# micahvista/VACmap

Hardware: AMD Instinct MI355X
Metric: aligned Gbp/s (whole node) + reads/s, 15 kb ONT-shape reads vs hg38-size ref, 1/2/4/8 MI355X (higher is better)
Workload: dtype i16/i32 DP + f64 chains

## Files before the change

### include/vacmapx.h

```cpp
#ifndef VACMAPX_H
#define VACMAPX_H
#include <stdint.h>
#ifdef __cplusplus
extern "C" {
#endif

typedef enum vm_status {
    VM_OK = 0,
    VM_ERR_ARG = -1,
    VM_ERR_NO_DEVICE = -2,
    VM_ERR_NO_CTX = -3,
    VM_ERR_OOM = -4,
    VM_ERR_IO = -5,
    VM_ERR_HIP = -6,
    VM_ERR_UNSUPPORTED = -7,
    VM_READ_RAISED = -10,
    VM_READ_CAPACITY = -20,
    VM_READ_FASTPATH = -21,
    VM_READ_UNSUPPORTED = -22
} vm_status;

enum { VM_MODE_H = 0, VM_MODE_L = 1, VM_MODE_S = 2, VM_MODE_R = 3,
       VM_MODE_ASM = 4 };

// ... 45 lines not shown
int vm_index_blob_count(const vm_index*);
int vm_index_blob(const vm_index*, int i, void** dev_ptr, int64_t* bytes);
int vm_index_meta_size(const vm_index*, int64_t* bytes);
int vm_index_meta_get(const vm_index*, void* buf, int64_t bytes);
int vm_index_from_meta(vm_ctx*, const void* buf, int64_t bytes, vm_index** out);

int vm_sketch_batch(vm_ctx*, int k, int w, int64_t n, const char* seqs, const int64_t* offsets,
                    uint64_t** hash, int32_t** pos, int8_t** strand, int64_t** off);
int vm_map_batch(vm_ctx*, const vm_index*, int check_num, int mid_occ, int64_t n, const char* seqs,
                 const int64_t* offsets, int64_t** anchors, int64_t** anchor_off);
int vm_map(vm_ctx*, const vm_index*, const char* seq, int64_t len, int check_num, int mid_occ, int64_t** anchors, int64_t* n);

typedef struct vm_chains_out {
    int32_t* need_reverse;
    int32_t* mapq;
    double* score;
    int32_t* fast_used;
    int64_t* read_path_off;
    int64_t* path_off;
    int64_t* path_anchors;
    double* S; int64_t* P; int64_t* S_arg; int64_t* gmax; int64_t* opcount;
} vm_chains_out;
int vm_chain_global_batch(vm_ctx*, const vm_params*, int kmersize, int64_t n, const int64_t* anchors,
                          const int64_t* anchor_off, const int64_t* readlens, int want_raw, vm_chains_out* out);
void vm_chains_out_free(vm_chains_out*);

typedef struct vm_local_out {
    int32_t* status;
    int32_t* variant;
    double* score;
    int64_t* chain_off;
    int64_t* chain;
    int64_t* raw_off;
    int64_t* raw;
} vm_local_out;
int vm_local_chain_batch(vm_ctx*, const vm_index*, const vm_params*, int64_t n, const char* seqs, const int64_t* offsets,
                         const int64_t* read_path_off, const int64_t* path_off, const int64_t* path_anchors, vm_local_out* out);
void vm_local_out_free(vm_local_out*);

typedef struct vm_linked_out {
    int64_t gmax, n_hot, n_cold, opcount; double cold_max;
    double* S; int64_t* P; int64_t* S_arg_hot;
    int32_t carry_status, saved; int64_t n_carry; double* carry_S; int64_t* carry_P; int64_t* carry_rows; double carry_g_max_scores; int64_t carry_prereadloc;
} vm_linked_out;
int vm_chain_linked(vm_ctx*, int which, int kmersize, double skipcost, int maxdiff, int maxgap, int64_t n, const int64_t* rows, int64_t n_pre,
                    const double* pre_S, const int64_t* pre_P, double g_max_scores, int64_t g_max_index, int64_t prereadloc, vm_linked_out* out);
void vm_linked_out_free(vm_linked_out*);

typedef struct vm_score { int32_t match, mismatch, o1, e1, o2, e2; } vm_score;
int vm_k_cigar_batch(vm_ctx*, const vm_score*, int eqx, int64_t n, const char* t, const int64_t* t_off, const char* q,
                     const int64_t* q_off, char** cigars, int64_t** cigar_off, int32_t** scores);
int vm_k_cigar_batch_banded(vm_ctx*, const vm_score*, int eqx, int64_t n, const char* t, const int64_t* t_off, const char* q,
                            const int64_t* q_off, char** cigars, int64_t** cigar_off, int32_t** band_flag, int64_t* stats);
int vm_k_extend_batch(vm_ctx*, int match, int mismatch, int o, int e, int bw, int zdrop, int64_t n, const char* t,
                      const int64_t* t_off, const char* q, const int64_t* q_off, int32_t** t_e, int32_t** q_e, int32_t** score);
typedef struct vm_cigar_out { char* cigar; int32_t q_e, t_e, score; } vm_cigar_out;
int vm_k_cigar(vm_ctx*, const char* t, int64_t tl, const char* q, int64_t ql, const vm_score* sc, int bw, int zdrop,
               int eqx, vm_cigar_out* out);
int vm_edit_distance_batch(vm_ctx*, int64_t n, const char* q, const int64_t* q_off, const char* t, const int64_t* t_off,
                           int64_t** dist);
int64_t vm_edit_distance(vm_ctx*, const char* q, int64_t ql, const char* t, int64_t tl);
int vm_edit_distance_bound_batch(vm_ctx*, int tier, int64_t n, const char* q, const int64_t* q_off, const char* t, const int64_t* t_off,
                                 int64_t** bound);

typedef struct vm_record {
    int32_t read_idx;
    int32_t contig;
    int32_t strand;
    int32_t mapq;
    int64_t q_st, q_en;
    int64_t r_st, r_en;
    int64_t cigar_off, cigar_len;
} vm_record;

typedef struct vm_batch_stats {
    int64_t n_reads, read_bases, n_minimizers, n_hits, n_anchors, n_local_hits, n_local_anchors;
    int64_t n_segments, n_ed_problems, ed_cells, n_ext_problems, ext_cells, n_dp_problems, dp_cells;
    int64_t n_records, cigar_bytes, aligned_bases, n_unmapped, n_failed;
    int64_t dp_string_bytes;
    double ms_total;
    double ms_stage[16];
    double ms_gapfill_fill;
    double ms_gapfill_trace;
    int64_t n_gapfill_launches;
    int64_t n_ed_full;
    int64_t n_ed_tier2;
    int64_t n_ed_tier1;
    int64_t n_dp_redo;
    int64_t dp_redo_tb_bytes;
    double ms_local_seed;
    double ms_cluster;
    int64_t n_host_syncs;
    int64_t n_local_general;
    int64_t n_ext_retries;
    int64_t n_batch_retries;
    int64_t n_dp_redo_wide;
    int64_t n_dp_redo_full;
} vm_batch_stats;

int vm_align_batch(vm_ctx*, const vm_index*, const vm_params*, int64_t n_reads, const char* seqs, const int64_t* offsets,
                   vm_record** recs, int64_t* n_recs, char** cigar_blob, int32_t* status_per_read, vm_batch_stats* stats);
typedef struct vm_reads vm_reads;
int vm_reads_upload(vm_ctx*, int64_t n_reads, const char* seqs, const int64_t* offsets, vm_reads** out);
int vm_reads_reupload(vm_ctx*, vm_reads*, int64_t n_reads, const char* seqs, const int64_t* offsets);
void vm_reads_free(vm_reads*);
int vm_align_resident(vm_ctx*, const vm_index*, const vm_params*, const vm_reads*, vm_record** recs, int64_t* n_recs,
                      char** cigar_blob, int32_t* status_per_read, vm_batch_stats* stats);

int vm_align_asm(vm_ctx*, const vm_index*, const vm_params* p, const char* contig, int64_t len, int64_t split_len, int64_t batch_anchors, int64_t window,
                 vm_record** recs, int64_t* n_recs, char** cigar_blob, int32_t* status);

int vm_align_trace(vm_ctx*, const vm_index*, const vm_params*, int64_t n_reads, const char* seqs, const int64_t* offsets, int stage,
                   int64_t** rows, int64_t** row_off);

typedef struct vm_sam_opts {
    int32_t md, shortcs, cigar2cg, markunbalancetra, hardclip, fakecigar;
    const char* rg_id;
    int32_t asm_mode;
} vm_sam_opts;
int vm_sam_emit(const vm_index*, const vm_sam_opts*, int64_t n_reads, const char* names, const int64_t* name_off, const char* seqs, const int64_t* seq_off,
                const char* quals, const int64_t* qual_off, const char* comments, const int64_t* com_off, const vm_record* recs, int64_t n_recs,
                const char* cigar_blob, const int32_t* status, int nthreads, char** text, int64_t** text_off, int64_t* n_lines, int64_t* n_skipped);
int vm_sam_emit_device(vm_ctx*, const vm_index*, const vm_sam_opts*, int64_t n_reads, const char* names, const int64_t* name_off, const char* seqs,
                       const int64_t* seq_off, const char* quals, const int64_t* qual_off, const vm_record* recs, int64_t n_recs, const char* cigar_blob,
                       const int32_t* status, char** text, int64_t** text_off, int64_t* n_lines, int64_t* n_skipped);
int vm_sam_emit_device_times(vm_ctx*, double* seconds3);
int64_t vm_blob_gather(const char* blob, const int64_t* off, const int64_t* idx, int64_t n, char* out, int64_t* out_off);
int64_t vm_blob_write_parts_mmap(int fd, int64_t file_off, const char* const* blobs, const int64_t* const* offs, const int32_t* part, const int64_t* idx, int64_t n, int nthreads);
int64_t vm_blob_gather_parts(const char* const* blobs, const int64_t* const* offs, const int32_t* part, const int64_t* idx, int64_t n, char* out);
void* vm_pinned_alloc(int64_t bytes, int device);
void vm_pinned_free(void* p);
int64_t vm_blob_write_parts(int fd, const char* const* blobs, const int64_t* const* offs, const int32_t* part, const int64_t* idx, int64_t n);
typedef struct vm_fastx vm_fastx;
int vm_fastx_open(const char* path, vm_fastx** out);
int vm_fastx_open_range(const char* path, int64_t begin, int64_t end, vm_fastx** out);
void vm_fastx_close(vm_fastx*);
int64_t vm_fastx_read(vm_fastx*, int64_t max_reads, int64_t max_bases, char** names, int64_t** name_off, char** seqs, int64_t** seq_off, char** quals,
                      int64_t** qual_off, char** comments, int64_t** com_off);

typedef struct vm_bam_writer vm_bam_writer;
int vm_bam_writer_create(vm_ctx*, const char* sam_header, int64_t len, vm_bam_writer** out);
void vm_bam_writer_free(vm_bam_writer*);
int vm_bam_header(vm_bam_writer*, char** out, int64_t* n);
int vm_bam_encode(vm_bam_writer*, const char* sam, int64_t len, char** out, int64_t* n);
int vm_bam_compress_parts(vm_bam_writer*, const char* const* blobs, const int64_t* const* offs, const int32_t* part, const int64_t* idx, int64_t n,
                          char** out, int64_t* n_out);
int vm_bgzf_compress(vm_ctx*, const void* in, int64_t n, char** out, int64_t* n_out);

int vm_bgzf_decompress(vm_ctx*, const void* in, int64_t n, char** out, int64_t* n_out);
typedef struct vm_bam_reader vm_bam_reader;
// ... 26 lines not shown
```

### vacmap_amd/csrc/k_dp.hip

```cpp
#include "vmx_device.h"
#include "vmx_kernels.h"

__device__ __forceinline__ int vmx_tcode(uint8_t c) { return c < 4 ? (int)c : 6; }


__global__ void k_encode(const char* __restrict__ in, uint8_t* __restrict__ out, int64_t n) {
    int64_t i = (int64_t)blockIdx.x * blockDim.x + threadIdx.x;
    int64_t stride = (int64_t)gridDim.x * blockDim.x;
    for (; i < n; i += stride) out[i] = vmx_code((uint8_t)in[i]);
}

#define VMX_EXT_RING 512
__global__ void __launch_bounds__(64) k_extend(const uint8_t* __restrict__ tcodes, const int64_t* __restrict__ t_off,
                                               const uint8_t* __restrict__ qcodes, const int64_t* __restrict__ q_off, int n_prob,
                                               int match, int mismatch, int o, int e, int bw_in, int zdrop,
                                               int32_t* __restrict__ out_te, int32_t* __restrict__ out_qe, int32_t* __restrict__ out_sc, const int32_t* __restrict__ n_ptr) {
    if (n_ptr) n_prob = *n_ptr;
    __shared__ int sH[3][VMX_EXT_RING];
    __shared__ int sE[2][VMX_EXT_RING];
    __shared__ int sF[2][VMX_EXT_RING];
    const int lane = vmx_lane();
    const int RM = VMX_EXT_RING - 1;
    for (int p = blockIdx.x; p < n_prob; p += gridDim.x) {
        const uint8_t* T = tcodes + t_off[p];
// ... 396 lines not shown
                if (ns == 2) VMX_ADW_RUN(2); else if (ns == 3) VMX_ADW_RUN(3); else VMX_ADW_RUN(4);
#undef VMX_ADW_RUN
                keepX = gX > 0 && vmx_ad_proven(scX, tlX0, qlX0, gX, match, o1, e1, o2, e2);
                keepY = gY > 0 && vmx_ad_proven(scY, tlY0, qlY0, gY, match, o1, e1, o2, e2);
            }
            if (lane == 0) {
                if (keepX) out_score[pX] = VMX_PK_FLAG;
                if (keepY) out_score[pY] = VMX_PK_FLAG;
                const int kept = (int)keepX + (int)keepY, full = 1 + (int)(pY >= 0) - kept;
                if (kept) atomicAdd(redo_cnt + 6, kept);
                if (full) atomicAdd(redo_cnt + 7, full);
            }
            if (!keepX || (pY >= 0 && !keepY)) __syncthreads();
            if (!keepX) vmx_gapfill_fill_one<SCORE>(tcodes, qcodes, probs, pX, match, mismatch, o1, e1, o2, e2, tb_pool, bnd_pool, out_score, lane, VMX_PK_FLAG, redo_pool);
            if (pY >= 0 && !keepY) vmx_gapfill_fill_one<SCORE>(tcodes, qcodes, probs, pY, match, mismatch, o1, e1, o2, e2, tb_pool, bnd_pool, out_score, lane, VMX_PK_FLAG, redo_pool);
        }
    }
    while (true) {
        int q0;
        if (order) { int v = 0; if (lane == 0) v = atomicAdd(counter, 4); q0 = vmx_bcast0(v); }
        else { q0 = static_next; static_next += 4 * (int)gridDim.x; }
        if (q0 >= n_prob) break;
        const int qg = q0 + (lane >> 4);
        const int pg = qg < n_prob ? (order ? order[qg] : qg) : -1;
        bool x4 = false, skip = false;
        {
            vmx_dp_prob pr; pr.tl = 0; pr.ql = 0; pr.t_off = 0; pr.q_off = 0; pr.tb_off = 0; pr.bnd_off = 0;
            if (pg >= 0) pr = probs[pg];
            skip = redo_pass && pg >= 0 && VMX_REDO_PK(pr.tl, pr.ql);
            x4 = pg >= 0 && !skip && pr.tl > 0 && pr.ql > 0 && VMX_DP16X4_OK(pr.tl, pr.ql);
            if (!SCORE && x4 && (lane & 15) == 0) out_score[pg] = 0;
            if (__any(x4))
                vmx_gapfill_fill16x4<SCORE>(tcodes + pr.t_off, qcodes + pr.q_off, x4 ? pr.tl : 0, x4 ? pr.ql : 0, match, mismatch, o1, e1, o2, e2, vmx_tb_ptr(tb_pool, redo_pool, pr.tb_off),
                                            bnd_pool + pr.bnd_off, &out_score[pg < 0 ? 0 : pg], lane);
        }
        for (int gk = 0; gk < 4; ++gk) {
            const int p = vmx_readlane(pg, 16 * gk);
            if (p < 0 || vmx_readlane((int)(x4 || skip), 16 * gk)) continue;
            vmx_gapfill_fill_one<SCORE>(tcodes, qcodes, probs, p, match, mismatch, o1, e1, o2, e2, tb_pool, bnd_pool, out_score, lane, 0, redo_pool);
        }
    }
}

__device__ __forceinline__ void vmx_gapfill_ad_pass(const uint8_t* __restrict__ tcodes, const uint8_t* __restrict__ qcodes, vmx_dp_prob* __restrict__ probs, int n_prob,
                                                   int match, int mismatch, int o1, int e1, int o2, int e2, uint8_t* __restrict__ tb_pool, int32_t* __restrict__ bnd_pool,
                                                   int32_t* __restrict__ out_score, const int32_t* __restrict__ order, const int32_t* __restrict__ range, int32_t* __restrict__ counter,
                                                   int32_t* __restrict__ redo_list, int32_t* __restrict__ redo_cnt, int ad_pct, unsigned long long* __restrict__ redo_bytes,
                                                   unsigned long long redo_cap, int tb_by_ns) {
    const int lane = vmx_lane();
    const int pct = ad_pct & 0xffff, pct_min = (ad_pct >> 16) & 0xffff;
    const bool ad_ok = vmx_ad_scores_ok(match, mismatch, o1, e1, o2, e2);
    const int n_head = range[0] < n_prob ? range[0] : n_prob;
    bool head = n_head > 0;
    while (true) {
        int pX = -1, pY = -1;
        if (head) {
            int q; { int v = 0; if (lane == 0) v = atomicAdd(counter + 1, 1); q = vmx_bcast0(v); }
            if (q >= n_head) { head = false; continue; }
            if (lane < 16) pX = order[q];
        } else {
            int q0; { int v = 0; if (lane == 0) v = atomicAdd(counter, 8); q0 = n_head + vmx_bcast0(v); }
            if (q0 >= n_prob) break;
            const int qX = q0 + 2 * (lane >> 4), qY = qX + 1;
            if (qX < n_prob) pX = order[qX];
            if (qY < n_prob) pY = order[qY];
        }
        vmx_dp_prob prX, prY;
        prX.tl = 0; prX.ql = 0; prX.t_off = 0; prX.q_off = 0; prX.tb_off = 0; prY = prX;
        if (pX >= 0) prX = probs[pX];
        if (pY >= 0) prY = probs[pY];
        const bool x4X = pX >= 0 && prX.tl > 0 && prX.ql > 0 && VMX_DP16X4_OK(prX.tl, prX.ql), x4Y = pY >= 0 && prY.tl > 0 && prY.ql > 0 && VMX_DP16X4_OK(prY.tl, prY.ql);
        const int nsX = x4X && ad_ok ? vmx_ad_ns(prX.tl, prX.ql, match, o1, e1, o2, e2, pct, pct_min) : 0, nsY = x4Y && ad_ok ? vmx_ad_ns(prY.tl, prY.ql, match, o1, e1, o2, e2, pct, pct_min) : 0;
        const int ns = vmx_uniform_i32(vmx_wave_max_i32(nsX > nsY ? nsX : nsY));
        bool keepX = false, keepY = false, triedX = false, triedY = false;
        if (ns > 0) {
            int dloX = 0, dloY = 0;
            const bool fitX = !tb_by_ns || VMX_AD_W(nsX) == VMX_AD_W(ns), fitY = !tb_by_ns || VMX_AD_W(nsY) == VMX_AD_W(ns);
            const int gX = (nsX > 0 && fitX) ? vmx_ad_geom(prX.tl, prX.ql, ns, &dloX) : 0, gY = (nsY > 0 && fitY) ? vmx_ad_geom(prY.tl, prY.ql, ns, &dloY) : 0;
            const int tlX = gX > 0 ? prX.tl : 0, qlX = gX > 0 ? prX.ql : 0, tlY = gY > 0 ? prY.tl : 0, qlY = gY > 0 ? prY.ql : 0;
            int scX = 0, scY = 0;
#define VMX_AD_RUN(NSV) vmx_gapfill_fill_ad<NSV>(tcodes + prX.t_off, qcodes + prX.q_off, tlX, qlX, dloX, tb_pool + prX.tb_off, tcodes + prY.t_off, qcodes + prY.q_off, tlY, qlY, dloY, \
                                                 tb_pool + prY.tb_off, match, mismatch, o1, e1, o2, e2, lane, scX, scY)
            if (ns == 1) VMX_AD_RUN(1); else if (ns == 2) VMX_AD_RUN(2); else if (ns == 3) VMX_AD_RUN(3); else VMX_AD_RUN(4);
#undef VMX_AD_RUN
            triedX = gX > 0; triedY = gY > 0;
            keepX = gX > 0 && vmx_ad_proven(scX, prX.tl, prX.ql, gX, match, o1, e1, o2, e2);
            keepY = gY > 0 && vmx_ad_proven(scY, prY.tl, prY.ql, gY, match, o1, e1, o2, e2);
        }
        if ((lane & 15) == 0) {
            if (x4X) {
                out_score[pX] = keepX ? VMX_AD_FLAG + ns : 0;
                if (!keepX) {
                    if (triedX) atomicAdd(redo_cnt + 3, 1);
                    const unsigned long long need = (unsigned long long)VMX_REDO_TB_BYTES(prX.tl, prX.ql), at = atomicAdd(redo_bytes, need);
                    if (at + need > redo_cap) { probs[pX].tl = 0; probs[pX].ql = 0; probs[pX].tb_off = 0; }
                    else { probs[pX].tb_off = -(int64_t)at - 1; redo_list[atomicAdd(redo_cnt, 1)] = pX; }
                }
            }
            if (x4Y) {
                out_score[pY] = keepY ? VMX_AD_FLAG + ns : 0;
                if (!keepY) {
                    if (triedY) atomicAdd(redo_cnt + 3, 1);
                    const unsigned long long need = (unsigned long long)VMX_REDO_TB_BYTES(prY.tl, prY.ql), at = atomicAdd(redo_bytes, need);
                    if (at + need > redo_cap) { probs[pY].tl = 0; probs[pY].ql = 0; probs[pY].tb_off = 0; }
                    else { probs[pY].tb_off = -(int64_t)at - 1; redo_list[atomicAdd(redo_cnt, 1)] = pY; }
                }
            }
        }
        for (int gk = 0; gk < 8; ++gk) {
            const int p = vmx_readlane((gk & 1) ? pY : pX, 16 * (gk >> 1));
            if (p < 0 || vmx_readlane((int)((gk & 1) ? x4Y : x4X), 16 * (gk >> 1))) continue;
            vmx_gapfill_fill_one<false>(tcodes, qcodes, probs, p, match, mismatch, o1, e1, o2, e2, tb_pool, bnd_pool, out_score, lane);
        }
    }
}

__global__ void __launch_bounds__(64) k_gapfill_fill(const uint8_t* __restrict__ tcodes, const uint8_t* __restrict__ qcodes,
                                                     const vmx_dp_prob* __restrict__ probs, int n_prob, int match, int mismatch,
                                                     int o1, int e1, int o2, int e2, uint8_t* __restrict__ tb_pool,
                                                     int32_t* __restrict__ bnd_pool, int32_t* __restrict__ out_score,
                                                     const int32_t* __restrict__ order, int32_t* __restrict__ counter) {
    vmx_gapfill_fill_body<true>(tcodes, qcodes, probs, n_prob, match, mismatch, o1, e1, o2, e2, tb_pool, bnd_pool, out_score, order, counter);
}
__global__ void __launch_bounds__(64, 4) k_gapfill_fill_ns(const uint8_t* __restrict__ tcodes, const uint8_t* __restrict__ qcodes,
                                                        vmx_dp_prob* __restrict__ probs, int n_prob, int match, int mismatch,
                                                        int o1, int e1, int o2, int e2, uint8_t* __restrict__ tb_pool,
                                                        int32_t* __restrict__ bnd_pool, int32_t* __restrict__ out_score,
                                                        const int32_t* __restrict__ order, const int32_t* __restrict__ range, int32_t* __restrict__ counter,
                                                        int32_t* __restrict__ redo_list, int32_t* __restrict__ redo_cnt, int ad_pct,
                                                        unsigned long long* __restrict__ redo_bytes, const int32_t* __restrict__ n_ptr,
                                                        unsigned long long redo_cap, int tb_by_ns) {
    if (n_ptr) n_prob = *n_ptr;
    vmx_gapfill_ad_pass(tcodes, qcodes, probs, n_prob, match, mismatch, o1, e1, o2, e2, tb_pool, bnd_pool, out_score, order, range, counter, redo_list, redo_cnt, ad_pct, redo_bytes, redo_cap, tb_by_ns);
}
__global__ void __launch_bounds__(64) k_gapfill_redo(const uint8_t* __restrict__ tcodes, const uint8_t* __restrict__ qcodes, const vmx_dp_prob* __restrict__ probs,
                                                     int match, int mismatch, int o1, int e1, int o2, int e2, uint8_t* __restrict__ tb_pool,
                                                     int32_t* __restrict__ bnd_pool, int32_t* __restrict__ out_score, int32_t* __restrict__ redo_list,
                                                     int32_t* __restrict__ redo_cnt, uint8_t* __restrict__ redo_pool) {
    vmx_gapfill_fill_body<false, true>(tcodes, qcodes, probs, 0, match, mismatch, o1, e1, o2, e2, tb_pool, bnd_pool, out_score, nullptr, nullptr, redo_list, redo_cnt, redo_pool);
}

__global__ void k_gapfill_trace(const uint8_t* __restrict__ tcodes, const uint8_t* __restrict__ qcodes,
                                const vmx_dp_prob* __restrict__ probs, int n_prob, int eqx, const uint8_t* __restrict__ tb_pool,
                                uint32_t* __restrict__ run_pool, char* __restrict__ cig_pool, int32_t* __restrict__ cig_len,
                                const int32_t* __restrict__ band_flag, const uint8_t* __restrict__ redo_pool, int spread, int32_t* __restrict__ cig_q,
                                const int32_t* __restrict__ n_ptr) {
    VMX_SETPRIO(3);
    if (n_ptr) n_prob = *n_ptr;
    const int gt = (int)(blockIdx.x * blockDim.x + threadIdx.x);
    if (spread > 1 && gt % spread) return;
    int p = spread > 1 ? gt / spread : gt;
    if (p >= n_prob) return;
    const vmx_dp_prob pr = probs[p];
    const uint8_t* T = tcodes + pr.t_off;
    const uint8_t* Q = qcodes + pr.q_off;
    const int tl = pr.tl, ql = pr.ql;
    const uint8_t* tb = vmx_tb_ptr(tb_pool, redo_pool, pr.tb_off);
    uint32_t* runs = run_pool + pr.run_off;
    char* cig = cig_pool + pr.cig_off;
    bool x4 = tl > 0 && ql > 0 && VMX_DP16X4_OK(tl, ql);
    bool pk = !x4 && tl > 0 && ql > 0 && VMX_DP16_OK(tl, ql);
    const int flag = (x4 && band_flag != nullptr) ? band_flag[p] : 0;
    const int ns = flag > VMX_AD_FLAG ? flag - VMX_AD_FLAG : 0;
    if (flag == VMX_PK_FLAG) { x4 = false; pk = true; }
    int dlo = 0;
    if (ns) vmx_ad_geom(tl, ql, ns, &dlo);
    const int AW = ns ? VMX_AD_W(ns) : 4;
// ... 68 lines not shown
```

### vacmap_amd/csrc/k_ed.hip

```cpp
#include "vmx_device.h"
#include "vmx_kernels.h"

__device__ __forceinline__ int vmx_size_class(long long s) {
    if (s < 0) return -1;
    if (s == 0) return 0;
    const int e = 63 - __clzll(s);
    const int m = (int)((e >= 2 ? s >> (e - 2) : s << (2 - e)) & 3);
    return (e << 2) | m;
}
__global__ void __launch_bounds__(1024) k_size_order(const int64_t* __restrict__ size, const int32_t* __restrict__ n_ptr, int64_t thresh,
                                                     int32_t* __restrict__ order, int32_t* __restrict__ range, int32_t* __restrict__ counters) {
    VMX_SETPRIO(3);
    __shared__ int s_hist[256];
    __shared__ int s_cur[256];
    __shared__ int s_long;
    const int n = *n_ptr;
    const int lane = vmx_lane();
    if (threadIdx.x < 256) s_hist[threadIdx.x] = 0;
    if (threadIdx.x == 0) s_long = 0;
    __syncthreads();
    int nl = 0;
    for (int i0 = 0; i0 < n; i0 += (int)blockDim.x) {
        const int i = i0 + (int)threadIdx.x;
        const long long s = i < n ? size[i] : -1;
        int b = vmx_size_class(s);
        if (s > thresh) ++nl;
        unsigned long long todo = __ballot(b >= 0);
        while (todo) {
            const int leader = __ffsll((unsigned long long)todo) - 1;
            const int b0 = vmx_readlane(b, leader);
            const unsigned long long same = __ballot(b == b0);
            if (lane == leader) atomicAdd(&s_hist[b0], __popcll(same));
            todo &= ~same;
        }
    }
    if (nl) atomicAdd(&s_long, nl);
    __syncthreads();
    if (threadIdx.x == 0) {
        int acc = 0;
        for (int b = 255; b >= 0; --b) { s_cur[b] = acc; acc += s_hist[b]; }
        range[0] = s_long; range[1] = acc;
        counters[0] = 0; counters[1] = 0; counters[2] = 0; counters[3] = 0;
    }
    __syncthreads();
    for (int i0 = 0; i0 < n; i0 += (int)blockDim.x) {
        const int i = i0 + (int)threadIdx.x;
        const long long s = i < n ? size[i] : -1;
        int b = vmx_size_class(s);
        unsigned long long todo = __ballot(b >= 0);
        while (todo) {
            const int leader = __ffsll((unsigned long long)todo) - 1;
            const int b0 = vmx_readlane(b, leader);
            const unsigned long long same = __ballot(b == b0);
            int base = 0;
            if (lane == leader) base = atomicAdd(&s_cur[b0], __popcll(same));
            base = vmx_readlane(base, leader);
            if (b == b0) order[base + __popcll(same & ((1ULL << lane) - 1ULL))] = i;
            todo &= ~same;
        }
    }
}

// ... 175 lines not shown
```

### vacmap_amd/csrc/vmx_align.hip

```cpp
#include "vmx_host.h"
#include "vmx_stage.h"
#include "vmx_select.h"
#include "vmx_ext_state.h"
#include "vmx_round.h"
#include <algorithm>
#include <cstdio>
#include <cstdlib>
#include <cstddef>
#include <cstring>
#include <string>

using namespace vmx;

__global__ void k_orient(const uint8_t* codes, const int64_t* roff, const double* gscore, int n_reads, uint8_t* ocodes);
__global__ void k_scan_i64(const int64_t* in, int64_t* out, int64_t n, int pow2_round);
__global__ void k_ext_phase(vmx_ext_args A, int phase);
__global__ void k_ed_anchor_bound(vmx_ext_args A, const int32_t* probread, const uint8_t* qpool, const int64_t* qoff, const uint8_t* tpool, const int64_t* toff,
                                  int64_t* ub_out);
__global__ void k_desc_lens(const vmx_pair_desc* desc, const int32_t* n_prob, int64_t* tl, int64_t* ql);
__global__ void k_gather(const vmx_pair_desc* desc, const int32_t* n_prob, const int32_t* prob_read, const uint8_t* ocodes, const int64_t* roff,
                         const uint8_t* ref, const int64_t* t_off, const int64_t* q_off, uint8_t* tpool, uint8_t* qpool, int64_t pool_cap, vmx_ext_read* er);
__global__ void k_prob_owner(const vmx_ext_read* er, int n_reads, int use_dp, int32_t* prob_read);
__global__ void k_dp_sizes(const vmx_pair_desc* desc, const int32_t* n_prob, int64_t* tb_sz, int64_t* bnd_sz, int64_t* run_sz, int64_t* cig_sz);
__global__ void k_dp_table(const vmx_pair_desc* desc, const int32_t* n_prob, const int64_t* t_off, const int64_t* q_off, const int64_t* tb_off,
// ... 90 lines not shown
    const bool rows_kernel = vmx_chain_rows_on() && rmode != 2;
    for (int64_t r = 0; r < n; ++r) {
        int64_t m = h_aoff[r + 1] - h_aoff[r]; const int64_t L = h_roff[r + 1] - h_roff[r];
        if (m <= 2) continue;
        if (prm->mode == VM_MODE_ASM && L >= 500000) { asm_long.push_back(r); continue; }
        if ((double)m / (double)L > 5.0) continue;
        int bk = NB; for (int q = 0; q < NB; ++q) if (m <= caps[q] && caps[q] <= gc_lds_max) { bk = q; break; }
        if (rows_kernel) bk = NB;
        lists[bk].push_back((int32_t)r);
    }
    {
        std::vector<int32_t> rl; int64_t rl_off[NB + 2];
        for (int q = 0; q <= NB; ++q) {
            std::stable_sort(lists[q].begin(), lists[q].end(), [&](int32_t a, int32_t b) { return h_aoff[a + 1] - h_aoff[a] > h_aoff[b + 1] - h_aoff[b]; });
            rl_off[q] = (int64_t)rl.size(); rl.insert(rl.end(), lists[q].begin(), lists[q].end());
        }
        VMX_TRY(vmx_push(c, B.rl, rl.data(), rl.size()));
        VMX_HIP(hipMemsetAsync(B.gmax.p, 0xff, 8 * (size_t)n, c->stream));
        { static const int64_t kUnsupported = -4; for (int64_t r : asm_long) VMX_HIP(hipMemcpyAsync(B.gmax.as<int64_t>() + r, &kUnsupported, 8, hipMemcpyHostToDevice, c->stream)); }
#ifndef VMX_EMU
        VMX_HIP(hipFuncSetAttribute((const void*)k_chain_global, hipFuncAttributeMaxDynamicSharedMemorySize, (int)((size_t)caps[NB - 1] * VMX_GC_BYTES_PER_ANCHOR + 64)));
#endif
        vmx_fork fk(c);
        for (int q = NB; q >= 0; --q) {
            int cnt = (int)lists[q].size(); if (!cnt) continue;
            int cap = q < NB ? caps[q] : 0; size_t shmem = (size_t)cap * VMX_GC_BYTES_PER_ANCHOR + 64;
            if (rows_kernel) {
                hipLaunchKernelGGL((vmx_chain_rows_win3() ? k_chain_global_rows_w3 : k_chain_global_rows), dim3((unsigned)((cnt + 3) / 4)), dim3(64), 0, fk.next(), B.sorted.as<vmx_anchor>(), B.aoff.as<int64_t>(),
                                   B.rl.as<int32_t>() + rl_off[q], cnt, c->tables, B.gap.as<double>(), prm->global_skipcost, prm->global_maxdiff, 1000, B.S.as<double>(),
                                   B.P.as<int32_t>(), B.SA.as<int32_t>(), B.cov.as<uint8_t>(), B.gmax.as<int64_t>(), B.opc.as<int64_t>(), rmode, B.fp.as<double>(), B.pp.as<double>(),
                                   vmx_chain_dbg());
                continue;
            }
            hipLaunchKernelGGL(k_chain_global, dim3((unsigned)cnt), dim3(64), shmem, fk.next(), B.sorted.as<vmx_anchor>(), B.aoff.as<int64_t>(),
                               B.rl.as<int32_t>() + rl_off[q], cnt, cap, c->tables, B.gap.as<double>(), prm->global_skipcost, prm->global_maxdiff, 1000, B.S.as<double>(),
                               B.P.as<int32_t>(), B.SA.as<int32_t>(), B.cov.as<uint8_t>(), B.gmax.as<int64_t>(), B.opc.as<int64_t>(), rmode, B.fp.as<double>(), B.pp.as<double>());
        }
        fk.join();
        vmx_chain_dbg_report(c->stream);
        VMX_TRY(B.si.reserve(4 * (size_t)(tot + 1))); VMX_TRY(B.tg.reserve(8 * (size_t)(tot + 1))); VMX_TRY(B.cntp.reserve(4 * (size_t)(total_bases + 50 * n + 64)));
        hipLaunchKernelGGL(k_chain_global_fast, dim3((unsigned)n), dim3(64), 0, c->stream, B.sorted.as<vmx_anchor>(), B.aoff.as<int64_t>(), (int)n, d_roff, c->tables,
                           B.gap.as<double>(), prm->global_skipcost, prm->global_maxdiff, 1000, B.S.as<double>(), B.P.as<int32_t>(), B.SA.as<int32_t>(), B.cov.as<uint8_t>(),
                           B.si.as<int32_t>(), B.tg.as<int64_t>(), B.cntp.as<int32_t>(), B.gmax.as<int64_t>(), d_ran, rmode, B.fp.as<double>(), B.pp.as<double>());
    }
    VMX_TRY(B.scr.reserve((size_t)stt + 64)); VMX_TRY(vmx_push(c, B.soff, soff.data(), (size_t)n + 1));
    VMX_TRY(B.res.reserve(16 * (size_t)(n + 2) + 64));
    double* d_gscore; int32_t* d_mapq; int32_t* d_np; vmx_res_ptrs(B, n, &d_gscore, &d_mapq, &d_np);
    VMX_TRY(B.plen.reserve(4 * (size_t)(tot + 1))); VMX_TRY(B.prow.reserve(sizeof(vmx_anchor) * (size_t)(tot + 1)));
    return vmx_launch_chain_select(c, n, h_aoff.data(), B.sellist, B.sorted.as<vmx_anchor>(), B.aoff.as<int64_t>(), B.lens.as<int64_t>(), B.S.as<double>(), B.P.as<int32_t>(), B.SA.as<int32_t>(),
                                   B.gmax.as<int64_t>(), B.flip.as<int32_t>(), prm->mode, B.scr.as<char>(), B.soff.as<int64_t>(), d_mapq, d_gscore, d_np, B.plen.as<int32_t>(), B.prow.as<vmx_anchor>());
}

void vmx_gapfill_chunk(vm_ctx* c, vmx_batch_bufs& B, const vm_score& sc, int ad_pct, int eqx, int p0, int64_t pn, const int32_t* n_ptr, int64_t tb_off0,
                       int32_t* ctl, int32_t* redo_list, int64_t redo_cap, hipEvent_t* ke) {
    int fill_waves = 16;
    if (const char* e = getenv("VMX_FILL_WAVES")) { const int v = atoi(e); if (v >= 1 && v <= 32) fill_waves = v; }
    static const int tr_spread = [] { const char* e = getenv("VMX_TRACE_SPREAD"); const int v = e ? atoi(e) : 1; return v >= 1 && v <= 64 ? v : 1; }();
    int32_t* d_range = ctl; int32_t* d_cnt = ctl + 4; int32_t* d_redo_cnt = ctl + 12;
    unsigned long long* d_redo_bytes = (unsigned long long*)(ctl + 16); int32_t* scratch = ctl + 32;
    uint8_t* tb_base = B.tb.as<uint8_t>() - tb_off0;
    vmx_dp_prob* probs = B.dptab.as<vmx_dp_prob>() + p0; int32_t* score = B.dpscore.as<int32_t>() + p0;
    const unsigned Gs = (unsigned)std::max<int64_t>(1, std::min<int64_t>((pn + 1023) / 1024, (int64_t)c->num_cu * 2));
    hipLaunchKernelGGL(k_size_hist, dim3(Gs), dim3(256), 0, c->stream, B.dpsz[0].as<int64_t>() + p0, n_ptr, (int64_t)((1LL << 42) - 1), scratch);
    hipLaunchKernelGGL(k_size_scatter, dim3(Gs), dim3(256), 0, c->stream, B.dpsz[0].as<int64_t>() + p0, n_ptr, (const int32_t*)scratch, scratch + 257, B.order.as<int32_t>(), d_range, d_cnt);
    if (ke) (void)hipEventRecord(ke[0], c->stream);
    {
        vmx_lowprio lp(c);
        hipLaunchKernelGGL(k_gapfill_fill_ns, dim3((unsigned)std::max<int64_t>(1, std::min<int64_t>(pn, (int64_t)c->num_cu * fill_waves))), dim3(64), 0, lp.stream(), B.tpool.as<uint8_t>(), B.qpool.as<uint8_t>(),
                           probs, (int)pn, sc.match, sc.mismatch, sc.o1, sc.e1, sc.o2, sc.e2, tb_base, B.bnd.as<int32_t>(), score, B.order.as<int32_t>(), d_range, d_cnt,
                           redo_list, d_redo_cnt, ad_pct, d_redo_bytes, n_ptr, (unsigned long long)redo_cap, 1);
        lp.join();
    }
    hipLaunchKernelGGL(k_gapfill_redo, dim3((unsigned)std::max<int64_t>(1, std::min<int64_t>(pn, (int64_t)c->num_cu * 4))), dim3(64), 0, c->stream, B.tpool.as<uint8_t>(), B.qpool.as<uint8_t>(),
                       probs, sc.match, sc.mismatch, sc.o1, sc.e1, sc.o2, sc.e2, tb_base, B.bnd.as<int32_t>(), score, redo_list, d_redo_cnt, B.tbredo.as<uint8_t>());
    if (ke) (void)hipEventRecord(ke[1], c->stream);
    hipLaunchKernelGGL(k_gapfill_trace, dim3((unsigned)std::max<int64_t>(1, (pn * tr_spread + 63) / 64)), dim3(64), 0, c->stream, B.tpool.as<uint8_t>(), B.qpool.as<uint8_t>(), probs, (int)pn, eqx,
                       tb_base, B.run.as<uint32_t>(), B.cig.as<char>(), B.ciglen.as<int32_t>() + p0, score, B.tbredo.as<uint8_t>(), tr_spread, B.cigq.as<int32_t>() + p0, n_ptr);
    if (ke) (void)hipEventRecord(ke[2], c->stream);
}

#define LAUNCH1D(kernel, n, ...) hipLaunchKernelGGL(kernel, dim3((unsigned)std::max<int64_t>(1, std::min<int64_t>(((n) + 255) / 256, 4096))), dim3(256), 0, c->stream, __VA_ARGS__)

__global__ void k_ext_geometry(const int32_t* la_cnt, const int64_t* roff, int n, int mul, int tmask, long long tdiv, long long capA, long long capS, long long capB, int64_t* coff3,
                               int64_t* soff2, int64_t* bloboff, int64_t* tot);
__global__ void k_scan_part_dev(const int64_t* in, int64_t* part, const int32_t* n_ptr);
__global__ void k_scan_apply_dev(const int64_t* in, int64_t* out, const int64_t* part_off, const int32_t* n_ptr);
__global__ void k_scan_part(const int64_t* in, int64_t* part, int64_t n, int64_t chunk);
__global__ void k_scan_apply(const int64_t* in, int64_t* out, const int64_t* part_off, int64_t n, int64_t chunk);

static int dev_scan(vm_ctx* c, vmx_batch_bufs& B, const int64_t* in, int64_t* out, int64_t n) {
    if (n <= 16384) { hipLaunchKernelGGL(k_scan_i64, dim3(1), dim3(256), 0, c->stream, in, out, n, 0); return 0; }
    int64_t chunk = (n + 511) / 512; const int64_t nb = (n + chunk - 1) / chunk;
    VMX_TRY(B.scanpart.reserve(8 * (size_t)(nb + 2))); VMX_TRY(B.scanoff.reserve(8 * (size_t)(nb + 2)));
    hipLaunchKernelGGL(k_scan_part, dim3((unsigned)nb), dim3(256), 0, c->stream, in, B.scanpart.as<int64_t>(), n, chunk);
    hipLaunchKernelGGL(k_scan_i64, dim3(1), dim3(256), 0, c->stream, B.scanpart.as<int64_t>(), B.scanoff.as<int64_t>(), nb, 0);
    hipLaunchKernelGGL(k_scan_apply, dim3((unsigned)nb), dim3(256), 0, c->stream, in, out, B.scanoff.as<int64_t>(), n, chunk);
    return 0;
}

static int dev_scan_dev(vm_ctx* c, vmx_batch_bufs& B, const int64_t* in, int64_t* out, const int32_t* n_ptr) {
    const int nb = 512;
    VMX_TRY(B.scanpart.reserve(8 * (size_t)(nb + 2))); VMX_TRY(B.scanoff.reserve(8 * (size_t)(nb + 2)));
    hipLaunchKernelGGL(k_scan_part_dev, dim3(nb), dim3(256), 0, c->stream, in, B.scanpart.as<int64_t>(), n_ptr);
    hipLaunchKernelGGL(k_scan_i64, dim3(1), dim3(256), 0, c->stream, B.scanpart.as<int64_t>(), B.scanoff.as<int64_t>(), (int64_t)nb, 0);
    hipLaunchKernelGGL(k_scan_apply_dev, dim3(nb), dim3(256), 0, c->stream, in, out, B.scanoff.as<int64_t>(), n_ptr);
    return 0;
}

static const vm_score gf_score = {2, -4, 4, 2, 24, 1};

static int ext_gather_round(vm_ctx* c, vmx_batch_bufs& B, const vm_index_view& ix, int64_t n, const uint8_t* d_ocodes, const int64_t* d_roff, int cur, int redo_only,
                            int64_t round_cap, int64_t pool_cap, int stat_slot, bool dp, int64_t tb_limit, const int64_t* caps = nullptr, int64_t* plan_out = nullptr, int ad_pct = 0) {
    (void)n; (void)redo_only; (void)round_cap;
    if (!B.roundpart.p) { VMX_TRY(B.roundpart.reserve(8 * (size_t)VMX_ROUND_PART_WORDS)); VMX_HIP(hipMemsetAsync(B.roundpart.p, 0, 8 * (size_t)VMX_ROUND_PART_WORDS, c->stream)); }
    vmx_round_args R; memset(&R, 0, sizeof R);
    R.desc = B.desc[cur].as<vmx_pair_desc>(); R.n_prob = c->rc_cur;
    R.off[0] = B.toff.as<int64_t>(); R.off[1] = B.qoff.as<int64_t>();
// ... 186 lines not shown
        VMX_TRY(vmx_push(c, L.la_off, L.h_la_off.data(), (size_t)n + 1));
        VMX_TRY(vmx_push(c, L.chain, chains.data(), chains.size()));
        VMX_TRY(vmx_push(c, L.chain_len, len32.data(), (size_t)n));
        VMX_TRY(vmx_push(c, L.status, zero.data(), (size_t)n));
        VMX_HIP(vmx_stream_sync(c));
        for (int e = 0; e < 3; ++e) VMX_HIP(hipEventRecord(ev[nev++], c->stream));
        return 0;
    };
    { const int rcf = preset ? front_preset() : front(); if (rcf < 0) return rcf; }

    std::vector<int64_t> coff3((size_t)n + 1), soff2((size_t)n + 1), bloboff((size_t)n + 1);
    auto pool = [&](int bit, int64_t x) -> int64_t { const int64_t y = x * c->ext_mul; return (tmask & bit) ? std::max<int64_t>(y / tdiv, 1) : y; };
    int64_t cA = 0, cS = 0, cB = 0, cS_full = 0;
    if (!fast_local) {
        for (int64_t r = 0; r < n; ++r) {
            const int64_t cl = L.h_la_cnt[r], len = h_roff[r + 1] - h_roff[r];
            coff3[r + 1] = coff3[r] + (cl > 0 ? pool(1, 3 * cl + 8) : 0); soff2[r + 1] = soff2[r] + (cl > 0 ? pool(2, cl + 2) : 0);
            bloboff[r + 1] = bloboff[r] + (cl > 0 ? ((pool(4, 3 * len + 64 * (cl / 2 + 2) + 56) + 7) & ~(int64_t)7) : 0);
            if (cl > 0) cS_full += cl + 2;
        }
        cA = coff3[n]; cS = soff2[n]; cB = bloboff[n];
        if (!preset && c->ext_mul == 1 && tmask == 0) {
            c->geo_cap[0] = std::max<long long>(c->geo_cap[0], cA); c->geo_cap[1] = std::max<long long>(c->geo_cap[1], cS); c->geo_cap[2] = std::max<long long>(c->geo_cap[2], cB);
            c->geo_cap[3] = std::max<long long>(c->geo_cap[3], cS_full);
            c->geo_valid = true;
        }
    } else {
        cA = c->geo_cap[0]; cS = c->geo_cap[1]; cB = c->geo_cap[2]; cS_full = c->geo_cap[3];
    }
    VMX_TRY(B.er.reserve(sizeof(vmx_ext_read) * (size_t)(n + 1)));
    if (!fast_local) { const vmx_push_req rq[3] = {{&B.coff3, coff3.data(), 8 * ((size_t)n + 1)}, {&B.soff2, soff2.data(), 8 * ((size_t)n + 1)}, {&B.bloboff, bloboff.data(), 8 * ((size_t)n + 1)}}; VMX_TRY(vmx_push_many(c, rq, 3)); }
    else {
        VMX_TRY(B.coff3.reserve(8 * ((size_t)n + 2))); VMX_TRY(B.soff2.reserve(8 * ((size_t)n + 2))); VMX_TRY(B.bloboff.reserve(8 * ((size_t)n + 2))); VMX_TRY(B.geotot.reserve(64));
        hipLaunchKernelGGL(k_ext_geometry, dim3(1), dim3(1024), 0, c->stream, L.la_cnt.as<int32_t>(), d_roff, (int)n, c->ext_mul, tmask, (long long)tdiv, (long long)cA, (long long)cS, (long long)cB,
                           B.coff3.as<int64_t>(), B.soff2.as<int64_t>(), B.bloboff.as<int64_t>(), B.geotot.as<int64_t>());
    }
    VMX_TRY(B.segA.reserve(sizeof(vmx_anchor) * (size_t)(cA + 1))); VMX_TRY(B.segA_s.reserve(sizeof(vmx_anchor) * (size_t)(cA + 1)));
    VMX_TRY(B.st.reserve(4 * (size_t)(cS + 1))); VMX_TRY(B.en.reserve(4 * (size_t)(cS + 1))); VMX_TRY(B.st_s.reserve(4 * (size_t)(cS + 1))); VMX_TRY(B.en_s.reserve(4 * (size_t)(cS + 1)));
    VMX_TRY(B.segprob.reserve(4 * (size_t)(cS + 1))); VMX_TRY(B.dup.reserve(4 * (size_t)(cS + 1)));
    const int64_t round_cap = pool(8, cS_full + 16);
    const int64_t pool_cap = pool(16, 6 * total_bases + (1 << 20));
    int64_t Lmax_b = 1; for (int64_t r = 0; r < n; ++r) Lmax_b = std::max(Lmax_b, h_roff[r + 1] - h_roff[r]);
    const int64_t carry_stride = preset ? 32768 : 2 * Lmax_b + 32768;
    const int64_t ed_wgs = std::min<int64_t>(c->num_cu, 64);
    VMX_TRY(B.desc[0].reserve(sizeof(vmx_pair_desc) * (size_t)round_cap)); VMX_TRY(B.desc[1].reserve(sizeof(vmx_pair_desc) * (size_t)round_cap));
    VMX_TRY(B.rcount.reserve(256)); VMX_HIP(hipMemsetAsync(B.rcount.p, 0, 256, c->stream)); c->rc_next = 0; c->rc_cur = B.rcount.as<int32_t>(); VMX_TRY(B.oflow.reserve(64)); VMX_TRY(B.probread.reserve(4 * (size_t)round_cap));
    VMX_TRY(B.tl.reserve(8 * (size_t)(round_cap + 1))); VMX_TRY(B.ql.reserve(8 * (size_t)(round_cap + 1))); VMX_TRY(B.toff.reserve(8 * (size_t)(round_cap + 1))); VMX_TRY(B.qoff.reserve(8 * (size_t)(round_cap + 1)));
    VMX_TRY(B.tpool.reserve((size_t)pool_cap + 64)); VMX_TRY(B.qpool.reserve((size_t)pool_cap + 64));
    VMX_TRY(B.edout.reserve(8 * (size_t)(round_cap + 1))); VMX_TRY(B.carry.reserve((size_t)VMX_ED_WAVES * (size_t)carry_stride * (size_t)ed_wgs * 3 + 64)); VMX_TRY(B.ext3.reserve(12 * (size_t)(round_cap + 1)));
    VMX_TRY(B.rec.reserve(sizeof(vm_record) * (size_t)(cS + 1))); VMX_TRY(B.blob.reserve((size_t)cB + 64)); VMX_TRY(B.reccoff.reserve(8 * (size_t)(cS + 1)));
    VMX_TRY(B.recclen.reserve(4 * (size_t)(cS + 1))); VMX_TRY(B.dupd.reserve((size_t)cB + 64));
    VMX_HIP(hipMemsetAsync(B.oflow.p, 0, 4, c->stream));
    VMX_TRY(B.statblk.reserve(2048)); VMX_HIP(hipMemsetAsync(B.statblk.p, 0, 2048, c->stream));
    const size_t gfctl_bytes = (size_t)2 * (VMX_MAX_CHUNKS + 1) * VMX_GF_SLOT * 4;
    VMX_TRY(B.gfctl.reserve(gfctl_bytes)); VMX_HIP(hipMemsetAsync(B.gfctl.p, 0, gfctl_bytes, c->stream));
    vmx_ext_args A; memset(&A, 0, sizeof A);
    A.n_reads = (int)n; A.nseq = ix.nseq; A.local_maxdiff = preset ? 50 : prm->local_maxdiff ; A.asm_long = preset ? 1 : 0; A.nodiscard = prm->nodiscard; A.hardclip = prm->hardclip; A.redo_only = 0; A.mode = prm->mode; A.maxdivergence = prm->maxdivergence;
    A.ocodes = B.ocodes.as<uint8_t>(); A.roff = d_roff; A.ref = ix.codes; A.coff = ix.coff;
    A.chain = L.chain.as<vmx_anchor>(); A.chain_len = L.chain_len.as<int32_t>(); A.la_off = L.la_off.as<int64_t>(); A.lstatus = L.status.as<int32_t>();
    A.gscore = d_gscore; A.mapq = d_mapq; A.er = B.er.as<vmx_ext_read>(); A.coff3 = B.coff3.as<int64_t>(); A.soff = B.soff2.as<int64_t>();
    A.segA = B.segA.as<vmx_anchor>(); A.st = B.st.as<int32_t>(); A.en = B.en.as<int32_t>(); A.segA_snap = B.segA_s.as<vmx_anchor>(); A.st_snap = B.st_s.as<int32_t>(); A.en_snap = B.en_s.as<int32_t>();
    A.seg_prob = B.segprob.as<int32_t>(); A.dup = B.dup.as<int32_t>(); A.round_count = B.rcount.as<int32_t>(); A.round_cap = round_cap; A.overflow = B.oflow.as<int32_t>(); A.prob_read = B.probread.as<int32_t>();
    A.ed_out = B.edout.as<int64_t>(); A.ext_te = B.ext3.as<int32_t>(); A.ext_qe = B.ext3.as<int32_t>() + round_cap;
    A.rec = B.rec.as<vm_record>(); A.rec_blob = B.blob.as<char>(); A.blob_off = B.bloboff.as<int64_t>(); A.rec_coff = B.reccoff.as<int64_t>(); A.rec_clen = B.recclen.as<int32_t>();
    A.dup_d = B.dupd.as<double>();
    const unsigned gridR = (unsigned)((n + 63) / 64);
    static const int ext_env = [] { const char* e = getenv("VMX_EXT_SPREAD"); const int v = e ? atoi(e) : 0; return v >= 1 && v <= 64 ? v : 0; }();
    static const int rec_env = [] { const char* e = getenv("VMX_REC_SPREAD"); const int v = e ? atoi(e) : 0; return v >= 1 && v <= 64 ? v : 0; }();
    const int ext_spread = ext_env ? ext_env : (c->inflight >= 2 ? 1 : 16), rec_spread = rec_env ? rec_env : (c->inflight >= 2 ? 1 : 4);
    const unsigned gridX = (unsigned)((n * ext_spread + 63) / 64), gridXR = (unsigned)((n * rec_spread + 63) / 64);
    static const bool ext_wave = [] { const char* e = getenv("VMX_EXT_WAVE"); return !(e && atoi(e) == 0); }();
    int cur = 0;
    auto phase = [&](int ph) { A.desc = B.desc[cur].as<vmx_pair_desc>(); A.desc_prev = B.desc[cur ^ 1].as<vmx_pair_desc>();
                               c->rc_cur = B.rcount.as<int32_t>() + (c->rc_next++ & 63); A.round_count = c->rc_cur;
                               const bool wv = ext_wave && (ph == 0 || ph == 3 || ph == 5);
                               A.spread = wv ? 64 : ext_spread; hipLaunchKernelGGL(k_ext_phase, dim3(wv ? (unsigned)n : gridX), dim3(64), 0, c->stream, A, ph);
                               if (trace && trace->stage == ph && !A.redo_only && trace->off.empty()) {
                                   std::vector<vmx_ext_read> er((size_t)n); std::vector<vmx_anchor> sa((size_t)cA + 1); std::vector<int32_t> st_((size_t)cS + 1), en_((size_t)cS + 1);
                                   (void)hipMemcpyAsync(er.data(), B.er.p, sizeof(vmx_ext_read) * (size_t)n, hipMemcpyDeviceToHost, c->stream);
                                   (void)hipMemcpyAsync(sa.data(), B.segA.p, sizeof(vmx_anchor) * (size_t)cA, hipMemcpyDeviceToHost, c->stream);
                                   (void)hipMemcpyAsync(st_.data(), B.st.p, 4 * (size_t)cS, hipMemcpyDeviceToHost, c->stream);
                                   (void)hipMemcpyAsync(en_.data(), B.en.p, 4 * (size_t)cS, hipMemcpyDeviceToHost, c->stream);
                                   (void)vmx_stream_sync(c);
                                   trace->off.assign(1, 0);
                                   for (int64_t r = 0; r < n; ++r) {
                                       if (er[(size_t)r].active && er[(size_t)r].status == 0)
                                           for (int sg = 0; sg < er[(size_t)r].nseg; ++sg)
                                               for (int t = st_[(size_t)(soff2[r] + sg)]; t < en_[(size_t)(soff2[r] + sg)]; ++t) {
                                                   const vmx_anchor& a = sa[(size_t)(coff3[r] + t)];
                                                   const int64_t row[5] = {sg, a.q, a.r, a.s, a.l}; trace->rows.insert(trace->rows.end(), row, row + 5);
                                               }
                                       trace->off.push_back((int64_t)trace->rows.size() / 5);
                                   }
                               } };
    int ext_rounds = 0;
    auto ext_round = [&](int redo_only) -> int {
        int rc = ext_gather_round(c, B, ix, n, B.ocodes.as<uint8_t>(), d_roff, cur, redo_only, round_cap, pool_cap, 1 + ext_rounds++, false, 0);
        if (rc < 0) return rc;
        hipLaunchKernelGGL(k_extend, dim3((unsigned)((int64_t)c->num_cu * 16)), dim3(64), 0, c->stream, B.tpool.as<uint8_t>(), B.toff.as<int64_t>(), B.qpool.as<uint8_t>(),
                           B.qoff.as<int64_t>(), 0, 2, -4, 4, 4, 100, 50, B.ext3.as<int32_t>(), B.ext3.as<int32_t>() + round_cap, B.ext3.as<int32_t>() + 2 * round_cap, c->rc_cur);
        cur ^= 1;
        return 0;
    };
    std::vector<int64_t> dp_tot(5, 0);
    static std::mutex ad_m; static struct { int pct = 0, floor = 20, hold = 0; } ad_tab[16][8];
    auto& adr = ad_tab[c->device & 15][prm->mode & 7];
    int ad_cur; { std::lock_guard<std::mutex> g(ad_m); if (adr.pct == 0) adr.pct = vmx_ad_pct_env(prm->mode) & 0xffff; ad_cur = adr.pct; }
    const bool ad_pinned = getenv("VMX_AD_PCT") != nullptr || getenv("VMX_AD_PCT_MIN") != nullptr;
    const int ad_pct = ad_pinned ? vmx_ad_pct_env(prm->mode) : (ad_cur | (std::max(20, ad_cur - 25) << 16));
    static const int64_t tb_chunk = [] { const char* e = getenv("VMX_TB_CHUNK_GB"); const double v = e ? atof(e) : 0.0; return v > 0.5 ? (int64_t)(v * (double)(1 << 30)) : (int64_t)VMX_TB_CHUNK; }();
    int gf_chunks[2] = {0, 0}; int64_t gf_redo_cap = 0;
    auto gf_chunk = [&](int pass, int q, int p0, int64_t pn, const int32_t* n_ptr, int64_t tb_off0) {
        int32_t* ctl = B.gfctl.as<int32_t>() + (size_t)(pass * (VMX_MAX_CHUNKS + 1) + q) * VMX_GF_SLOT;
        hipEvent_t* ke = q < 8 ? c->gev + (pass ? 24 : 0) + 3 * q : nullptr;
        vmx_gapfill_chunk(c, B, gf_score, ad_pct, prm->eqx, p0, pn, n_ptr, tb_off0, ctl, B.order.as<int32_t>() + round_cap + 32, gf_redo_cap, ke);
        if (ke) c->n_gev[pass] = q + 1;
        gf_chunks[pass] = q + 1;
    };
    auto gapfill = [&](int redo_only) -> int {
        for (int i = 0; i < 4; ++i) { VMX_TRY(B.dpsz[i].reserve(8 * (size_t)(round_cap + 2))); VMX_TRY(B.dpoff[i].reserve(8 * (size_t)(round_cap + 2))); }
        VMX_TRY(B.dptab.reserve(sizeof(vmx_dp_prob) * (size_t)(round_cap + 1))); VMX_TRY(B.ciglen.reserve(4 * (size_t)(round_cap + 1))); VMX_TRY(B.cigq.reserve(4 * (size_t)(round_cap + 1))); VMX_TRY(B.dpscore.reserve(4 * (size_t)(round_cap + 1)));
        VMX_TRY(B.order.reserve(4 * (size_t)(2 * round_cap + 64)));
        if (!redo_only) {
            gf_redo_cap = std::max<int64_t>((int64_t)((double)c->redo_need_max * 1.3), std::min<int64_t>((int64_t)512 << 20, std::max<int64_t>(tb_chunk / 8, 1 << 20)));
            if (const char* e = getenv("VMX_TEST_REDO_POOL_BYTES")) { const long long v = atoll(e); if (v > 0 && c->redo_need_max == 0) gf_redo_cap = v; }
            VMX_TRY(B.tbredo.reserve((size_t)gf_redo_cap + 64));
            gf_redo_cap = (int64_t)B.tbredo.cap - 64;
        }
        c->n_gev[redo_only ? 1 : 0] = 0;
        {
            int rcg = ext_gather_round(c, B, ix, n, B.ocodes.as<uint8_t>(), d_roff, cur, redo_only, round_cap, pool_cap, 6 + redo_only, true, tb_chunk, nullptr, B.statblk.as<int64_t>() + 64 + (redo_only ? 64 : 0), ad_pct);
            if (rcg < 0) return rcg;
            int64_t plan[8 + 2 * (VMX_MAX_CHUNKS + 1)];
            VMX_TRY(vmx_fetch(c, plan, B.statblk.as<int64_t>() + 64 + (redo_only ? 64 : 0), sizeof(plan) / 8));
            VMX_HIP(vmx_stream_sync(c));
            const int cnt = (int)plan[0];
            int64_t totals[4] = {plan[1], plan[2], plan[3], plan[4]};
            if (plan[7] < 0) { set_error("gap fill: more traceback chunks than VMX_MAX_CHUNKS"); return VM_ERR_OOM; }
            st.n_dp_problems += cnt; st.dp_cells += totals[0]; st.dp_string_bytes += plan[5] + plan[6];
            std::vector<int32_t> cuts; std::vector<int64_t> h_tboff_at;
            for (int q = 0; q <= (int)plan[7]; ++q) { cuts.push_back((int32_t)plan[8 + q]); h_tboff_at.push_back(plan[8 + VMX_MAX_CHUNKS + 1 + q]); }
            if (cuts.size() < 2) { cuts.assign(2, 0); h_tboff_at.assign(2, 0); }
            int64_t tbmax = 0;
            for (size_t q = 0; q + 1 < cuts.size(); ++q) tbmax = std::max(tbmax, h_tboff_at[q + 1] - h_tboff_at[q]);
            VMX_TRY(B.tb.reserve((size_t)tbmax + 64)); VMX_TRY(B.bnd.reserve(4 * (size_t)(totals[1] + 4))); VMX_TRY(B.run.reserve(4 * (size_t)(totals[2] + 4))); VMX_TRY(B.cig.reserve((size_t)totals[3] + 16));
            if (cnt) {
                std::vector<int32_t> csz; for (size_t q = 0; q + 1 < cuts.size(); ++q) csz.push_back(cuts[q + 1] - cuts[q]);
                VMX_TRY(vmx_push(c, B.chunkn, csz.data(), csz.size()));
                for (size_t q = 0; q + 1 < cuts.size(); ++q) gf_chunk(redo_only, (int)q, cuts[q], cuts[q + 1] - cuts[q], B.chunkn.as<int32_t>() + q, h_tboff_at[q]);
            }
        }
        A.redo_only = redo_only;
        A.spread = rec_spread;
        hipLaunchKernelGGL(k_ext_records, dim3((unsigned)n), dim3(64), 0, c->stream, A, B.dptab.as<vmx_dp_prob>(), B.cig.as<char>(), B.ciglen.as<int32_t>(), B.cigq.as<int32_t>());
        cur ^= 1;
        return 0;
    };
    phase(0);
    {
        int rc0 = ext_gather_round(c, B, ix, n, B.ocodes.as<uint8_t>(), d_roff, cur, 0, round_cap, pool_cap, 0, false, 0);
        if (rc0 < 0) return rc0;
        const int64_t cnt = round_cap;
        {
            VMX_TRY(B.order.reserve(4 * (size_t)(2 * round_cap + 64))); VMX_TRY(B.qrange.reserve(128)); VMX_TRY(B.szh.reserve(4 * 520));
            int32_t* d_range = B.qrange.as<int32_t>(); int32_t* d_cnt = d_range + 4; int32_t* d_nfull = d_range + 8;
            VMX_TRY(B.dpsz[0].reserve(8 * (size_t)(round_cap + 2))); VMX_TRY(B.dpsz[1].reserve(8 * (size_t)(round_cap + 2)));
            int32_t* d_n2 = d_range + 9; int32_t* d_n1 = d_range + 10;
            (void)hipMemsetAsync(d_nfull, 0, 12, c->stream);
// ... 14 lines not shown
                               B.tpool.as<uint8_t>(), B.toff.as<int64_t>(), B.order.as<int32_t>(), d_range, d_cnt + 2, B.dpsz[1].as<int64_t>());
            hipLaunchKernelGGL(k_ed_flag, dim3((unsigned)std::min<int64_t>((cnt + 255) / 256, 1024)), dim3(256), 0, c->stream, B.dpsz[1].as<int64_t>(), B.qoff.as<int64_t>(), B.toff.as<int64_t>(),
                               c->rc_cur, prm->maxdivergence, B.dpsz[0].as<int64_t>(), B.edout.as<int64_t>(), d_nfull, 0, (const int32_t*)nullptr, (vmx_ext_read*)nullptr);
            vmx_size_order_wide(c, B.dpsz[0].as<int64_t>(), c->rc_cur, cnt, (int64_t)VMX_ED_LONG, B.order.as<int32_t>(), d_range, d_cnt, B.szh.as<int32_t>());
            for (int which = 0; which < 2; ++which)
                hipLaunchKernelGGL(k_edit_distance, dim3((unsigned)std::min<int64_t>(cnt, ed_wgs * (which == 0 ? 1 : 2))), dim3(which == 0 ? 64 * VMX_ED_WAVES : 256), 0, c->stream,
                                   B.qpool.as<uint8_t>(), B.qoff.as<int64_t>(), B.tpool.as<uint8_t>(), B.toff.as<int64_t>(),
                                   B.carry.as<int8_t>() + (which ? (size_t)VMX_ED_WAVES * (size_t)carry_stride * (size_t)ed_wgs : 0), B.order.as<int32_t>(), d_range, d_cnt, which,
                                   B.edout.as<int64_t>(), carry_stride, B.oflow.as<int32_t>());
            }
        }
        cur ^= 1;
    }
    VMX_HIP(hipEventRecord(ev[nev++], c->stream));
    phase(1); VMX_TRY(ext_round(0));
    phase(2); VMX_TRY(ext_round(0));
    phase(3); VMX_TRY(ext_round(0));
    phase(4); VMX_TRY(ext_round(0));
    VMX_HIP(hipEventRecord(ev[nev++], c->stream));
    phase(5); VMX_TRY(gapfill(0));
    VMX_HIP(hipEventRecord(ev[nev++], c->stream));
    int64_t test_side_every = 0; if (const char* e = getenv("VMX_TEST_SIDE_EVERY")) test_side_every = atoll(e);
    static const bool always_pass1 = getenv("VMX_FORCE_PASS1") != nullptr;
    const bool do_pass1 = c->run_pass1 || always_pass1;
    if (do_pass1) {
        A.redo_only = 1;
        phase(3); phase(4); phase(5); VMX_TRY(gapfill(1));
        A.redo_only = 0;
    }
    VMX_HIP(hipEventRecord(ev[nev++], c->stream));

    VMX_TRY(B.dpsz[0].reserve(8 * (size_t)(n + 2))); VMX_TRY(B.dpsz[1].reserve(8 * (size_t)(n + 2))); VMX_TRY(B.dpoff[0].reserve(8 * (size_t)(n + 2))); VMX_TRY(B.dpoff[1].reserve(8 * (size_t)(n + 2)));
    hipLaunchKernelGGL(k_res_sizes, dim3(gridR), dim3(64), 0, c->stream, B.er.as<vmx_ext_read>(), B.rec.as<vm_record>(), B.soff2.as<int64_t>(), (int)n, B.dpsz[0].as<int64_t>(), B.dpsz[1].as<int64_t>());
    hipLaunchKernelGGL(k_scan_i64, dim3(1), dim3(256), 0, c->stream, B.dpsz[0].as<int64_t>(), B.dpoff[0].as<int64_t>(), n, 0);
    hipLaunchKernelGGL(k_scan_i64, dim3(1), dim3(256), 0, c->stream, B.dpsz[1].as<int64_t>(), B.dpoff[1].as<int64_t>(), n, 0);
    int64_t nr = 0, nb = 0; int32_t oflow = 0;
    int32_t n_full = 0, n_t2 = 0, n_t1 = 0;
    int64_t fin[14]; int64_t hstat[8];
    hipLaunchKernelGGL(k_final_scalars, dim3(1), dim3(1), 0, c->stream, B.dpoff[0].as<int64_t>() + n, B.dpoff[1].as<int64_t>() + n, B.oflow.as<int32_t>(), B.qrange.as<int32_t>() + 8,
                       B.statblk.as<int32_t>(), B.statblk.as<int64_t>() + 32);
    VMX_TRY(B.totals.reserve(sizeof(vm_record) * (size_t)(cS + 1))); VMX_TRY(B.dupd.reserve((size_t)cB + 64));
    hipLaunchKernelGGL(k_res_pack, dim3((unsigned)std::min<int64_t>(n, (int64_t)c->num_cu * 8)), dim3(64), 0, c->stream, B.er.as<vmx_ext_read>(), B.rec.as<vm_record>(), B.blob.as<char>(),
                       B.soff2.as<int64_t>(), B.bloboff.as<int64_t>(), (int)n, B.dpoff[0].as<int64_t>(), B.dpoff[1].as<int64_t>(), B.totals.as<vm_record>(), B.dupd.as<char>());
    int64_t g_nr = std::min<int64_t>(cS, (int64_t)(c->res_rec_per_read * 2.0 * (double)n) + 256), g_nb = std::min<int64_t>(cB, (int64_t)(c->res_blob_per_base * 1.5 * (double)total_bases) + 65536);
    if (c->res_rec_per_read <= 0.0) { g_nr = 0; g_nb = 0; }
    std::vector<vmx_ext_read> er((size_t)n);
    std::vector<int64_t> h_gmax((size_t)n);
    *recs = (vm_record*)malloc(sizeof(vm_record) * (size_t)std::max<int64_t>(g_nr, 1)); *cigar_blob = (char*)malloc((size_t)std::max<int64_t>(g_nb, 1));
    struct OutGuard { vm_record** r; char** b; bool keep = false; ~OutGuard() { if (!keep) { free(*r); free(*b); *r = nullptr; *b = nullptr; } } } out_guard{recs, cigar_blob};
    if (!*recs || !*cigar_blob) { set_error("out of host memory"); return VM_ERR_OOM; }
    VMX_TRY(vmx_fetch(c, fin, B.statblk.as<int64_t>() + 32, 14));
    int64_t geo[8] = {0, 0, 0, 0, 0, 0, 0, 0};
    if (fast_local) VMX_TRY(vmx_fetch(c, geo, B.geotot.p, 6));
    std::vector<int32_t> h_ctl(gfctl_bytes / 4);
    VMX_TRY(vmx_fetch(c, h_ctl.data(), B.gfctl.p, h_ctl.size()));
    VMX_TRY(vmx_fetch(c, er.data(), B.er.p, (size_t)n)); VMX_TRY(vmx_fetch(c, h_gmax.data(), B.gmax.p, (size_t)n));
    VMX_TRY(vmx_fetch(c, *recs, B.totals.p, (size_t)g_nr)); VMX_TRY(vmx_fetch(c, *cigar_blob, B.dupd.p, (size_t)g_nb));
    VMX_HIP(hipEventRecord(ev[nev++], c->stream));
    VMX_HIP(vmx_stream_sync(c));
    VMX_HIP(hipGetLastError());
    nr = fin[0]; nb = fin[1]; oflow = (int32_t)fin[2]; n_full = (int32_t)fin[3]; n_t2 = (int32_t)fin[4]; n_t1 = (int32_t)fin[5];
    if (fast_local) {
        st.n_local_anchors = geo[4];
        if (geo[5] > 0 || geo[3] + 16 > c->geo_cap[3]) c->geo_valid = false;
        if (geo[5] && getenv("VMX_DBG_POOLS")) fprintf(stderr, "[pools] extend stage: %lld read(s) did not fit the history-sized pools (run again alone)\n", (long long)geo[5]);
    }
    {
        bool again = false; int64_t need_max = 0, ad_failed = 0;
        for (int pass = 0; pass < 2; ++pass)
            for (int q = 0; q < gf_chunks[pass]; ++q) {
                const int32_t* ctl = h_ctl.data() + (size_t)(pass * (VMX_MAX_CHUNKS + 1) + q) * VMX_GF_SLOT;
                unsigned long long rb = 0; memcpy(&rb, ctl + 16, 8);
                st.n_dp_redo += ctl[12]; st.n_dp_redo_wide += ctl[18]; st.n_dp_redo_full += ctl[19]; st.dp_redo_tb_bytes += (int64_t)rb; st.dp_cells += (int64_t)rb; ad_failed += ctl[15];
                need_max = std::max<int64_t>(need_max, (int64_t)rb);
            }
        c->redo_need_max = std::max<long long>(c->redo_need_max, need_max);
        if (need_max > gf_redo_cap) { again = true; if (getenv("VMX_DBG_POOLS")) fprintf(stderr, "[pools] gap fill: a chunk's second launch needs %.3f GB of traceback space, the pool held %.3f: running the batch again\n", need_max / 1e9, gf_redo_cap / 1e9); }
        if (again) return VMX_RETRY_BATCH;
        if (!ad_pinned && !c->force_exact && st.n_dp_problems >= 2000) {
            const double f = (double)ad_failed / (double)st.n_dp_problems;
            std::lock_guard<std::mutex> g(ad_m);
            if (ad_cur == adr.pct) {
                if (f > 0.03 && adr.pct < 100) { adr.pct = std::min(100, adr.pct + 10); adr.floor = adr.pct; adr.hold = 256; }
                else if (adr.hold > 0) { if (--adr.hold == 0) adr.floor = 20; }
                else if (f < 0.025 && adr.pct > adr.floor) adr.pct = std::max(adr.floor, adr.pct - (f < 0.01 ? 20 : 10));
            }
        }
    }
    for (int i = 0; i < 8; ++i) hstat[i] = fin[6 + i];
    st.n_segments = hstat[0]; st.n_ed_problems = hstat[0]; st.n_ext_problems = (int64_t)hstat[1] + hstat[2] + hstat[3] + hstat[4];
    st.n_ed_full = n_full; st.n_ed_tier2 = n_t2; st.n_ed_tier1 = n_t1;
    if (oflow) { set_error("extend stage: a per-batch work pool overflowed"); return VM_ERR_OOM; }
    if (nr > g_nr || nb > g_nb) {
        if (nr > g_nr) { vm_record* p2 = (vm_record*)realloc(*recs, sizeof(vm_record) * (size_t)nr); if (!p2) { set_error("out of host memory"); return VM_ERR_OOM; } *recs = p2;
                         VMX_TRY(vmx_fetch(c, *recs + g_nr, B.totals.as<vm_record>() + g_nr, (size_t)(nr - g_nr))); }
        if (nb > g_nb) { char* p2 = (char*)realloc(*cigar_blob, (size_t)nb); if (!p2) { set_error("out of host memory"); return VM_ERR_OOM; } *cigar_blob = p2;
                         VMX_TRY(vmx_fetch(c, *cigar_blob + g_nb, B.dupd.as<char>() + g_nb, (size_t)(nb - g_nb))); }
        VMX_HIP(vmx_stream_sync(c));
    }
    if (n > 0 && total_bases > 0) { c->res_rec_per_read = std::max(c->res_rec_per_read, (double)nr / (double)n); c->res_blob_per_base = std::max(c->res_blob_per_base, (double)nb / (double)total_bases); }
    for (int64_t r = 0; r < n; ++r) {
        int stt2 = er[r].status == VMX_EXT_CAPACITY_DEV ? VMX_EXT_SHORT_INTERNAL : (er[r].status == VMX_EXT_NEED_EXACT_DEV ? VMX_EXT_EXACT_INTERNAL : er[r].status);
        if (fast_local && (er[r].status == VM_READ_CAPACITY_DEV || er[r].status == VM_READ_BANDFALL_DEV)) stt2 = VMX_EXT_EXACT_INTERNAL;
        if (stt2 == 0 && !do_pass1 && er[r].active && er[r].redo == 1 && er[r].pass == 1) stt2 = VMX_EXT_EXACT_INTERNAL;
        if (stt2 == 0 && test_side_every > 0 && !c->force_exact && r % test_side_every == 0) stt2 = VMX_EXT_EXACT_INTERNAL;
        if (h_gmax[r] == -2 && (h_aoff[r + 1] - h_aoff[r]) > 2) stt2 = VM_READ_RAISED;
        if (h_gmax[r] == -4) stt2 = VM_READ_UNSUPPORTED;
        if (!asm_override.empty() && asm_override[(size_t)r] != 0) stt2 = asm_override[(size_t)r];
        if (rmode == 1 && (h_aoff[r + 1] - h_aoff[r]) <= 2) stt2 = VM_READ_RAISED;
        if (status_per_read) status_per_read[r] = stt2;
        if (stt2 != 0) { st.n_failed++; continue; }
        if (er[r].nrec == 0) st.n_unmapped++;
    }
    for (int64_t i = 0; i < nr; ++i) { st.aligned_bases += (*recs)[i].q_en - (*recs)[i].q_st; st.cigar_bytes += (*recs)[i].cigar_len; }
    *n_recs = nr; st.n_records = nr;
    float ms = 0;
    hipEventElapsedTime(&ms, ev[0], ev[nev - 1]); st.ms_total = ms;
    for (int i = 1; i < nev && i < 16; ++i) { hipEventElapsedTime(&ms, ev[i - 1], ev[i]); st.ms_stage[i - 1] = ms; }
    if ((c->kev_set & 1) && hipEventElapsedTime(&ms, c->kev[0], c->kev[1]) == hipSuccess) st.ms_local_seed = ms;
    if ((c->kev_set & 2) && hipEventElapsedTime(&ms, c->kev[2], c->kev[3]) == hipSuccess) st.ms_cluster = ms;
    st.n_host_syncs = c->n_syncs; st.n_local_general = c->n_bandfall;
    st.ms_stage[14] = (float)((c->sync_wait_ns + download_wait_ns()) * 1e-6);
    st.ms_stage[15] = (float)((std::chrono::duration_cast<std::chrono::nanoseconds>(std::chrono::steady_clock::now().time_since_epoch()).count() - c->call_t0_ns) * 1e-6);
    for (int pass = 0; pass < 2; ++pass)
        for (int q = 0; q < c->n_gev[pass]; ++q) {
            hipEvent_t* ke = c->gev + 24 * pass + 3 * q;
            if (hipEventElapsedTime(&ms, ke[0], ke[1]) == hipSuccess) st.ms_gapfill_fill += ms;
            if (hipEventElapsedTime(&ms, ke[1], ke[2]) == hipSuccess) st.ms_gapfill_trace += ms;
// ... 3 lines not shown
    if (getenv("VMX_DBG_POOLS")) {
        const DevBuf* bb = (const DevBuf*)&B; size_t tot = 0;
        for (size_t i = 0; i < sizeof(B) / sizeof(DevBuf); ++i) { tot += bb[i].cap; if (bb[i].cap > ((size_t)128 << 20)) fprintf(stderr, "[pools] batch[%zu] %.2f GB\n", i, bb[i].cap / 1e9); }
        fprintf(stderr, "[pools] batch bufs total %.2f GB\n", tot / 1e9);
        const DevBuf* lb = (const DevBuf*)&L; size_t lt = 0; const size_t nl = (size_t)((const char*)&L.la_pool_rows - (const char*)&L) / sizeof(DevBuf);
        for (size_t i = 0; i < nl; ++i) { lt += lb[i].cap; if (lb[i].cap > ((size_t)128 << 20)) fprintf(stderr, "[pools] local[%zu] %.2f GB\n", i, lb[i].cap / 1e9); }
        fprintf(stderr, "[pools] local bufs total %.2f GB\n", lt / 1e9);
        fprintf(stderr, "[pools] process so far: %lld first allocations, %lld re-allocations, %.3f s in hipFree + hipMalloc\n", (long long)vmx::devbuf_stats().first.load(),
                (long long)vmx::devbuf_stats().grows.load(), vmx::devbuf_stats().ns.load() * 1e-9);
    }
    if (stats) *stats = st;
    out_guard.keep = true;
    return VM_OK;
}

template <class RunOne>
static int align_in_sub_batches(int64_t n, const int64_t* offsets, int64_t max_bases, RunOne run_one, vm_record** recs, int64_t* n_recs, char** cigar_blob, vm_batch_stats* stats) {
    if (n <= VMX_MAX_BATCH_READS && offsets[n] - offsets[0] <= max_bases) {
        const int rc = run_one(0, n, recs, n_recs, cigar_blob, stats);
        if (rc != VM_ERR_OOM || n <= 1) return rc;
        free(*recs); free(*cigar_blob);
    }
    *recs = nullptr; *n_recs = 0; *cigar_blob = nullptr;
    std::vector<vm_record> all; std::string blob;
    vm_batch_stats tot; memset(&tot, 0, sizeof tot);
    std::vector<std::pair<int64_t, int64_t>> work;
    for (int64_t a = 0; a < n;) {
        int64_t b = a + 1;
        while (b < n && b - a < VMX_MAX_BATCH_READS && offsets[b + 1] - offsets[a] <= max_bases) ++b;
        work.emplace_back(a, b); a = b;
    }
    for (size_t wi = 0; wi < work.size(); ++wi) {
        const int64_t a = work[wi].first, b = work[wi].second;
        vm_record* r = nullptr; int64_t nr = 0; char* cb = nullptr; vm_batch_stats st;
        const int rc = run_one(a, b, &r, &nr, &cb, &st);
        if (rc == VM_ERR_OOM && b - a > 1) {
            free(r); free(cb);
            vmx::devbuf_retired().flush();
            const int64_t mid = a + (b - a) / 2;
            work[wi] = std::make_pair(a, mid); work.insert(work.begin() + (std::ptrdiff_t)wi + 1, std::make_pair(mid, b));
            --wi; continue;
        }
        if (rc < 0) { free(r); free(cb); return rc; }
        int64_t bl = 0; for (int64_t i = 0; i < nr; ++i) bl = std::max(bl, r[i].cigar_off + r[i].cigar_len);
        for (int64_t i = 0; i < nr; ++i) { vm_record x = r[i]; x.read_idx += (int32_t)a; x.cigar_off += (int64_t)blob.size(); all.push_back(x); }
        blob.append(cb, (size_t)bl); blob.push_back('\0');
        free(r); free(cb);
        {
            int64_t* d = (int64_t*)&tot; const int64_t* s2 = (const int64_t*)&st;
            for (size_t i = 0; i < offsetof(vm_batch_stats, ms_total) / 8; ++i) d[i] += s2[i];
            tot.ms_total += st.ms_total; for (int i = 0; i < 16; ++i) tot.ms_stage[i] += st.ms_stage[i];
            tot.ms_gapfill_fill += st.ms_gapfill_fill; tot.ms_gapfill_trace += st.ms_gapfill_trace; tot.n_gapfill_launches += st.n_gapfill_launches;
            tot.n_ed_full += st.n_ed_full; tot.n_ed_tier2 += st.n_ed_tier2; tot.n_ed_tier1 += st.n_ed_tier1;
            tot.n_dp_redo += st.n_dp_redo; tot.n_dp_redo_wide += st.n_dp_redo_wide; tot.n_dp_redo_full += st.n_dp_redo_full; tot.dp_redo_tb_bytes += st.dp_redo_tb_bytes; tot.ms_local_seed += st.ms_local_seed; tot.ms_cluster += st.ms_cluster; tot.n_host_syncs += st.n_host_syncs; tot.n_local_general += st.n_local_general; tot.n_ext_retries += st.n_ext_retries; tot.n_batch_retries += st.n_batch_retries;
        }
    }
    *recs = (vm_record*)malloc(sizeof(vm_record) * std::max<size_t>(all.size(), 1)); *cigar_blob = (char*)malloc(std::max<size_t>(blob.size(), 1));
    if (!*recs || !*cigar_blob) { free(*recs); free(*cigar_blob); *recs = nullptr; *cigar_blob = nullptr; set_error("out of host memory"); return VM_ERR_OOM; }
    memcpy(*recs, all.data(), sizeof(vm_record) * all.size()); memcpy(*cigar_blob, blob.data(), blob.size());
    *n_recs = (int64_t)all.size();
    if (stats) *stats = tot;
    return VM_OK;
}
static int64_t vmx_pass_bases() {
    static const int64_t v = [] { const char* e = getenv("VMX_MAX_BATCH_BASES"); const long long x = e ? atoll(e) : 0; return x > 0 ? (int64_t)x : (int64_t)VMX_MAX_BATCH_BASES; }();
    return v;
}

extern "C" {

int vm_reads_upload(vm_ctx* c, int64_t n, const char* seqs, const int64_t* offsets, vm_reads** out) {
    *out = nullptr;
    if (!c) { set_error("no context"); return VM_ERR_NO_CTX; }
    VMX_HIP(hipSetDevice(c->device));
    vm_reads* R = new vm_reads(); R->ctx = c; R->n = n; R->h_off.assign(offsets, offsets + n + 1);
    const int64_t tot = offsets[n];
    int rc = 0;
    if ((rc = upload(R->raw, seqs, (size_t)tot, c->stream)) < 0 || (rc = R->codes.reserve((size_t)tot + 64)) < 0 || (rc = upload(R->off, offsets, (size_t)n + 1, c->stream)) < 0) { delete R; return rc; }
    if (tot) LAUNCH1D(k_encode, tot, R->raw.as<char>(), R->codes.as<uint8_t>(), tot);
    VMX_HIP(vmx_stream_sync(c));
    R->raw.release();
    *out = R;
    return VM_OK;
}
int vm_reads_reupload(vm_ctx* c, vm_reads* R, int64_t n, const char* seqs, const int64_t* offsets) {
    if (!c || !R) { set_error("no context / reads object"); return VM_ERR_NO_CTX; }
    VMX_HIP(hipSetDevice(c->device));
    R->n = n; R->h_off.assign(offsets, offsets + n + 1);
    const int64_t tot = offsets[n];
    VMX_TRY(upload(R->raw, seqs, (size_t)tot, c->stream)); VMX_TRY(R->codes.reserve((size_t)tot + 64)); VMX_TRY(upload(R->off, offsets, (size_t)n + 1, c->stream));
    if (tot) LAUNCH1D(k_encode, tot, R->raw.as<char>(), R->codes.as<uint8_t>(), tot);
    VMX_HIP(vmx_stream_sync(c));
    return VM_OK;
}
void vm_reads_free(vm_reads* R) { if (!R) return; R->raw.release(); R->codes.release(); R->off.release(); delete R; }

int vm_align_resident(vm_ctx* c, const vm_index* mi, const vm_params* prm, const vm_reads* R, vm_record** recs, int64_t* n_recs, char** cigar_blob,
                      int32_t* status_per_read, vm_batch_stats* stats) {
    if (!c) { set_error("no context"); return VM_ERR_NO_CTX; }
    VMX_HIP(hipSetDevice(c->device));
    if (R->n <= VMX_MAX_BATCH_READS && R->h_off[(size_t)R->n] <= vmx_pass_bases())
        return align_device(c, mi, prm, R->n, R->codes.as<uint8_t>(), R->off.as<int64_t>(), R->h_off, recs, n_recs, cigar_blob, status_per_read, stats);
    vmx_batch_bufs& B = *vmx_ctx_batch_bufs(c);
    auto run_one = [&](int64_t a, int64_t b, vm_record** r, int64_t* nr, char** cb, vm_batch_stats* st) -> int {
        std::vector<int64_t> h((size_t)(b - a) + 1);
        for (int64_t i = a; i <= b; ++i) h[(size_t)(i - a)] = R->h_off[(size_t)i] - R->h_off[(size_t)a];
        VMX_TRY(vmx_push(c, B.off, h.data(), h.size()));
// ... 56 lines not shown
```

### vacmap_amd/csrc/vmx_capi.hip

```cpp
#include "vmx_host.h"
#include <time.h>
#include "vmx_select.h"
#include "vmx_stage.h"
#include "vmx_round.h"
#include <algorithm>
#include <cmath>
#include <cstdlib>
#include <cstring>
#include <numeric>

namespace vmx {
static thread_local std::string g_err;
void set_error(const std::string& s) { g_err = s; }
int hip_fail(hipError_t e, const char* what, const char* file, int line) {
    g_err = std::string("HIP error: ") + hipGetErrorString(e) + " at " + what + " (" + file + ":" + std::to_string(line) + ")";
    return e == hipErrorOutOfMemory ? VM_ERR_OOM : VM_ERR_HIP;
}
}
using namespace vmx;

void vmx_ctx_free_local_bufs(vm_ctx* c);
void vmx_ctx_free_batch_bufs(vm_ctx* c);
void vmx_ctx_free_sam_bufs(vm_ctx* c);

// ... 463 lines not shown
    }
    VMX_TRY(upload(c->b[6], probs.data(), (size_t)n, c->stream));
    VMX_TRY(c->b[7].reserve((size_t)tb + 64)); VMX_TRY(c->b[8].reserve(sizeof(int32_t) * (size_t)(bnd + 4)));
    VMX_TRY(c->b[9].reserve(sizeof(uint32_t) * (size_t)(run + 4))); VMX_TRY(c->b[10].reserve((size_t)cig + 16));
    VMX_TRY(c->b[11].reserve(sizeof(int32_t) * 2 * (size_t)(n + 1)));
    int32_t* d_score = c->b[11].as<int32_t>(); int32_t* d_len = d_score + n;
    if (n) {
        hipLaunchKernelGGL(k_gapfill_fill, dim3(grid_for(c, n, 16)), dim3(64), 0, c->stream, c->b[1].as<uint8_t>(), c->b[4].as<uint8_t>(),
                           c->b[6].as<vmx_dp_prob>(), (int)n, sc->match, sc->mismatch, sc->o1, sc->e1, sc->o2, sc->e2, c->b[7].as<uint8_t>(),
                           c->b[8].as<int32_t>(), d_score, (const int32_t*)nullptr, (int32_t*)nullptr);
        hipLaunchKernelGGL(k_gapfill_trace, dim3((unsigned)((n + 63) / 64)), dim3(64), 0, c->stream, c->b[1].as<uint8_t>(), c->b[4].as<uint8_t>(),
                           c->b[6].as<vmx_dp_prob>(), (int)n, eqx, c->b[7].as<uint8_t>(), c->b[9].as<uint32_t>(), c->b[10].as<char>(), d_len, (const int32_t*)nullptr, (const uint8_t*)nullptr, 1, (int32_t*)nullptr);
    }
    std::vector<char> hc((size_t)cig + 16); std::vector<int32_t> hl((size_t)n);
    *scores = host_alloc<int32_t>((size_t)n);
    VMX_TRY(download(hc.data(), c->b[10].p, (size_t)cig, c->stream));
    VMX_TRY(download(hl.data(), d_len, (size_t)n, c->stream));
    VMX_TRY(download(*scores, d_score, (size_t)n, c->stream));
    VMX_HIP(hipStreamSynchronize(c->stream));
    VMX_HIP(hipGetLastError());
    cigar_strings(n, probs.data(), hc.data(), hl.data(), cigars, cigar_off);
    return VM_OK;
}

int vm_k_cigar_batch_banded(vm_ctx* c, const vm_score* sc, int eqx, int64_t n, const char* t, const int64_t* t_off, const char* q,
                            const int64_t* q_off, char** cigars, int64_t** cigar_off, int32_t** band_flag, int64_t* stats) {
    if (!c) { set_error("no context"); return VM_ERR_NO_CTX; }
    if (n > 0x7fffffff) { set_error("too many problems"); return VM_ERR_ARG; }
    VMX_HIP(hipSetDevice(c->device));
    vmx_fetch_scope fetch_scope(c);
    vmx_batch_bufs& B = *vmx_ctx_batch_bufs(c);
    VMX_TRY(upload_encode(c, t, t_off, n, c->b[0], B.tpool, c->b[2]));
    VMX_TRY(upload_encode(c, q, q_off, n, c->b[3], B.qpool, c->b[5]));
    const int ad_pct = vmx_ad_pct_env();
    vmx_round_args R; memset(&R, 0, sizeof R);
    R.ad_on = 1; R.ad_match = sc->match; R.ad_o1 = sc->o1; R.ad_e1 = sc->e1; R.ad_o2 = sc->o2; R.ad_e2 = sc->e2; R.ad_pct = ad_pct;
    std::vector<vmx_dp_prob> probs((size_t)n);
    std::vector<int64_t> keys((size_t)n);
    int64_t tb = 0, bnd = 0, run = 0, cig = 0, redo = 0;
    for (int64_t i = 0; i < n; ++i) {
        vmx_dp_prob& p = probs[i];
        p.t_off = t_off[i]; p.q_off = q_off[i]; p.tl = (int32_t)(t_off[i + 1] - t_off[i]); p.ql = (int32_t)(q_off[i + 1] - q_off[i]);
        p.tb_off = tb; p.bnd_off = bnd; p.run_off = run; p.cig_off = cig;
        tb += vmx_round_tb_bytes(R, p.tl, p.ql); keys[i] = vmx_round_key(R, p.tl, p.ql);
        if (p.tl > 0 && p.ql > 0 && VMX_DP16X4_OK(p.tl, p.ql)) redo += VMX_REDO_TB_BYTES((int64_t)p.tl, (int64_t)p.ql);
        bnd += 3 * (int64_t)(p.ql + 1); run += (int64_t)p.tl + p.ql + 2; cig += 2 * ((int64_t)p.tl + p.ql) + 16;
    }
    const int32_t nn = (int32_t)n;
    VMX_TRY(upload(B.dptab, probs.data(), (size_t)n, c->stream)); VMX_TRY(upload(B.dpsz[0], keys.data(), (size_t)n, c->stream)); VMX_TRY(upload(B.chunkn, &nn, 1, c->stream));
    VMX_TRY(B.tb.reserve((size_t)tb + 64)); VMX_TRY(B.tbredo.reserve((size_t)redo + 64)); VMX_TRY(B.bnd.reserve(sizeof(int32_t) * (size_t)(bnd + 4)));
    VMX_TRY(B.run.reserve(sizeof(uint32_t) * (size_t)(run + 4))); VMX_TRY(B.cig.reserve((size_t)cig + 16));
    VMX_TRY(B.ciglen.reserve(4 * (size_t)(n + 1))); VMX_TRY(B.cigq.reserve(4 * (size_t)(n + 1))); VMX_TRY(B.dpscore.reserve(4 * (size_t)(n + 1)));
    VMX_TRY(B.order.reserve(4 * (size_t)(2 * n + 64)));
    VMX_TRY(B.gfctl.reserve(4 * VMX_GF_SLOT)); VMX_HIP(hipMemsetAsync(B.gfctl.p, 0, 4 * VMX_GF_SLOT, c->stream));
    if (n) vmx_gapfill_chunk(c, B, *sc, ad_pct, eqx, 0, n, B.chunkn.as<int32_t>(), 0, B.gfctl.as<int32_t>(), B.order.as<int32_t>() + n + 32, redo, nullptr);
    std::vector<char> hc((size_t)cig + 16); std::vector<int32_t> hl((size_t)n), flag((size_t)n), ctl(32);
    VMX_TRY(download(hc.data(), B.cig.p, (size_t)cig, c->stream));
    VMX_TRY(download(hl.data(), B.ciglen.p, (size_t)n, c->stream));
    VMX_TRY(download(flag.data(), B.dpscore.p, (size_t)n, c->stream));
    VMX_TRY(download(ctl.data(), B.gfctl.p, ctl.size(), c->stream));
    VMX_HIP(vmx_stream_sync(c));
    VMX_HIP(hipGetLastError());
    int64_t nb = 0, eligible = 0, small = 0;
    for (int64_t i = 0; i < n; ++i) {
        const bool sm = probs[i].tl > 0 && probs[i].ql > 0 && VMX_DP16X4_OK(probs[i].tl, probs[i].ql);
        if (!sm) flag[i] = 0;
        small += sm; nb += sm && flag[i] > VMX_AD_FLAG;
        eligible += sm && vmx_ad_ns(probs[i].tl, probs[i].ql, sc->match, sc->o1, sc->e1, sc->o2, sc->e2, ad_pct & 0xffff, (ad_pct >> 16) & 0xffff) > 0;
    }
    if (stats) { stats[0] = eligible; stats[1] = nb; stats[2] = ctl[12]; stats[3] = n - small; stats[4] = ctl[18]; stats[5] = ctl[19]; }
    if (band_flag) { *band_flag = host_alloc<int32_t>((size_t)n); memcpy(*band_flag, flag.data(), sizeof(int32_t) * (size_t)n); }
    cigar_strings(n, probs.data(), hc.data(), hl.data(), cigars, cigar_off);
    return VM_OK;
}

int vm_k_cigar(vm_ctx* c, const char* t, int64_t tl, const char* q, int64_t ql, const vm_score* sc, int bw, int zdrop, int eqx, vm_cigar_out* out) {
    memset(out, 0, sizeof(*out));
    int64_t to[2] = {0, tl}, qo[2] = {0, ql};
    if (zdrop < 0) {
        char* cg = nullptr; int64_t* co = nullptr; int32_t* s = nullptr;
        int rc = vm_k_cigar_batch(c, sc, eqx, 1, t, to, q, qo, &cg, &co, &s);
        if (rc < 0) return rc;
        out->cigar = cg; out->q_e = (int32_t)ql; out->t_e = (int32_t)tl; out->score = s[0];
        free(co); free(s);
        return VM_OK;
    }
    if (sc->o1 != sc->o2 || sc->e1 != sc->e2) { set_error("vm_k_cigar: z-drop extension needs identical gap pieces (the reference calls it with 4,4,4,4)"); return VM_ERR_UNSUPPORTED; }
    int32_t *te = nullptr, *qe = nullptr, *s = nullptr;
    int rc = vm_k_extend_batch(c, sc->match, sc->mismatch, sc->o1, sc->e1, bw, zdrop, 1, t, to, q, qo, &te, &qe, &s);
    if (rc < 0) return rc;
    out->cigar = (char*)calloc(1, 1); out->t_e = te[0]; out->q_e = qe[0]; out->score = s[0];
    free(te); free(qe); free(s);
    return VM_OK;
}

void vm_chains_out_free(vm_chains_out* o) {
    free(o->need_reverse); free(o->mapq); free(o->score); free(o->fast_used); free(o->read_path_off); free(o->path_off);
    free(o->path_anchors); free(o->S); free(o->P); free(o->S_arg); free(o->gmax); free(o->opcount);
    memset(o, 0, sizeof(*o));
}

int vm_chain_global_batch(vm_ctx* c, const vm_params* prm, int kmersize, int64_t n, const int64_t* anchors, const int64_t* aoff,
                          const int64_t* readlens, int want_raw, vm_chains_out* out) {
    memset(out, 0, sizeof(*out));
    if (!c) { set_error("no context"); return VM_ERR_NO_CTX; }
    if (prm->global_maxdiff > 62) { set_error("global_maxdiff > 62 unsupported"); return VM_ERR_UNSUPPORTED; }
    const int64_t tot = aoff[n];
    if (const int64_t bad = vmx_rows_misfit(anchors, tot); bad >= 0) {
        char msg[192]; snprintf(msg, sizeof msg, "vm_chain_global_batch: anchor row %lld does not fit the device row (l in 0 ... 65535, q and q + l in int32, s in int16)", (long long)bad);
        set_error(msg); return VM_ERR_UNSUPPORTED;
    }
    VMX_HIP(hipSetDevice(c->device));
    vmx_fetch_scope fetch_scope(c);
    vmx_batch_bufs& B = *vmx_ctx_batch_bufs(c);
    const std::vector<int64_t> h_aoff(aoff, aoff + n + 1);
    std::vector<int64_t> h_roff((size_t)n + 1, 0);
    for (int64_t r = 0; r < n; ++r) h_roff[(size_t)r + 1] = h_roff[(size_t)r] + readlens[r];
    VMX_TRY(upload(B.rows, anchors, (size_t)tot * 4, c->stream)); VMX_TRY(upload(B.aoff, aoff, (size_t)n + 1, c->stream));
    VMX_TRY(upload(B.lens, readlens, (size_t)n, c->stream)); VMX_TRY(upload(B.off, h_roff.data(), (size_t)n + 1, c->stream));
    DevBuf& d_ran = c->b[0];
    VMX_TRY(d_ran.reserve(4 * (size_t)(n + 1))); VMX_HIP(hipMemsetAsync(d_ran.p, 0, 4 * (size_t)n, c->stream));
    const int rmode = prm->mode == VM_MODE_R ? 1 : (prm->mode == VM_MODE_ASM ? 2 : 0);
    double* d_score = nullptr; int32_t* d_mapq = nullptr; int32_t* d_np = nullptr;
    if (n) {
        VMX_TRY(vmx_global_stage(c, B, prm, kmersize, n, B.off.as<int64_t>(), h_roff, h_aoff, rmode, d_ran.as<int32_t>()));
        vmx_res_ptrs(B, n, &d_score, &d_mapq, &d_np);
// ... 44 lines not shown
```

### vacmap_amd/csrc/vmx_device.h

```cpp
#ifndef VMX_DEVICE_H
#define VMX_DEVICE_H
#ifdef VMX_EMU
#include "hip_emu.h"
#define VMX_DYN_SHARED(type, name) type* name = (type*)hipemu::cur()->dynshared
#else
#include <hip/hip_runtime.h>
#define VMX_DYN_SHARED(type, name) extern __shared__ __attribute__((aligned(16))) type name[]
#endif
#include <stdint.h>

#define VMX_WAVE 64
#define VMX_NEG (-(1 << 28))
#define VMX_NOPRE (-9999999)

__device__ __forceinline__ int vmx_lane() { return (int)(threadIdx.x & 63); }

#ifdef VMX_EMU
__device__ __forceinline__ int vmx_shr1(int v) { return __shfl_up(v, 1); }
__device__ __forceinline__ int vmx_readlane(int v, int l) { return __shfl(v, l); }
#define VMX_SPIN_PAUSE() hipemu::yield()
#define VMX_CLOCK() 0LL
#else
__device__ __forceinline__ int vmx_shr1(int v) { return __builtin_amdgcn_update_dpp(v, v, 0x138, 0xf, 0xf, false); }
__device__ __forceinline__ int vmx_readlane(int v, int l) { return __builtin_amdgcn_readlane(v, l); }
// ... 53 lines not shown
#endif
#ifdef VMX_EMU
__device__ __forceinline__ void vmx_wave_lds_fence() { __syncthreads(); }
#else
__device__ __forceinline__ void vmx_wave_lds_fence() { asm volatile("" ::: "memory"); }
#endif
__device__ __forceinline__ unsigned vmx_bfi(unsigned m, unsigned a, unsigned b) { return (m & a) | (~m & b); }
#ifdef VMX_EMU
__device__ __forceinline__ int vmx_uniform_i32(int v) { return v; }
#else
__device__ __forceinline__ int vmx_uniform_i32(int v) { return __builtin_amdgcn_readfirstlane(v); }
#endif
__device__ __forceinline__ long long vmx_uniform_i64(long long v) {
    union { long long d; int i[2]; } u; u.d = v;
    u.i[0] = vmx_uniform_i32(u.i[0]); u.i[1] = vmx_uniform_i32(u.i[1]);
    return u.d;
}
__device__ __forceinline__ double vmx_uniform_f64(double v) {
    union { double d; int i[2]; } u; u.d = v;
    u.i[0] = vmx_uniform_i32(u.i[0]); u.i[1] = vmx_uniform_i32(u.i[1]);
    return u.d;
}
#ifdef VMX_EMU
#define VMX_GLOBAL_PTR(T, p) (p)
#else
#define VMX_GLOBAL_PTR(T, p) ((T*)(__attribute__((address_space(1))) T*)(unsigned long long)vmx_uniform_i64((long long)(p)))
#endif
#ifdef VMX_EMU
__device__ __forceinline__ int vmx_bcast0(int v) { return __shfl(v, 0); }
#else
__device__ __forceinline__ int vmx_bcast0(int v) { return __builtin_amdgcn_readfirstlane(v); }
#endif
__device__ __forceinline__ double vmx_shr1_f64(double v) {
    union { double d; int i[2]; } u; u.d = v;
    u.i[0] = vmx_shr1(u.i[0]); u.i[1] = vmx_shr1(u.i[1]);
    return u.d;
}
__device__ __forceinline__ long long vmx_shr1_i64(long long v) {
    union { long long d; int i[2]; } u; u.d = v;
    u.i[0] = vmx_shr1(u.i[0]); u.i[1] = vmx_shr1(u.i[1]);
    return u.d;
}
struct vmx_cwin { int j, q, ls; double S; long long r; };
__device__ __forceinline__ void vmx_cwin_insert(vmx_cwin& w, int at, int k, double Sk, int qk, int lsk, long long rk, int lane) {
    const int sj = vmx_shr1(w.j), sq = vmx_shr1(w.q), sls = vmx_shr1(w.ls);
    const double sS = vmx_shr1_f64(w.S); const long long sr = vmx_shr1_i64(w.r);
    if (lane > at) { w.j = sj; w.q = sq; w.ls = sls; w.S = sS; w.r = sr; }
    else if (lane == at) { w.j = k; w.q = qk; w.ls = lsk; w.S = Sk; w.r = rk; }
}
__device__ __forceinline__ double vmx_readlane_f64(double v, int l) {
    union { double d; int i[2]; } u; u.d = v;
    u.i[0] = vmx_readlane(u.i[0], l); u.i[1] = vmx_readlane(u.i[1], l);
    return u.d;
}

__device__ __forceinline__ int vmx_wave_max_i32(int v) {
    for (int o = 32; o > 0; o >>= 1) { int x = __shfl_xor(v, o); v = x > v ? x : v; }
    return v;
}
__device__ __forceinline__ int vmx_wave_sum_i32(int v) {
    for (int o = 32; o > 0; o >>= 1) v += __shfl_xor(v, o);
    return v;
}
__device__ __forceinline__ long long vmx_wave_sum_i64(long long v) {
    for (int o = 32; o > 0; o >>= 1) v += __shfl_xor(v, o);
    return v;
}
__device__ __forceinline__ int vmx_wave_incl_scan_i32(int v) {
    int lane = vmx_lane();
    for (int o = 1; o < 64; o <<= 1) { int x = __shfl_up(v, o); if (lane >= o) v += x; }
    return v;
}
__device__ __forceinline__ double vmx_wave_excl_max_f64(double v, double init) {
    int lane = vmx_lane();
    for (int o = 1; o < 64; o <<= 1) { double x = __shfl_up(v, o); if (lane >= o) v = x > v ? x : v; }
    double e = __shfl_up(v, 1);
    if (lane == 0) e = init; else e = e > init ? e : init;
    return e;
}

#define VMX_F64_NEG (-__builtin_inf())
#ifdef VMX_EMU
__device__ __forceinline__ double vmx_wave_incl_max_f64(double v) {
    int lane = vmx_lane();
    for (int o = 1; o < 64; o <<= 1) { double x = __shfl_up(v, o); if (lane >= o) v = x > v ? x : v; }
    return v;
}
__device__ __forceinline__ double vmx_wave_shr1_f64_fill(double v, double fill) {
    double e = __shfl_up(v, 1);
    return vmx_lane() == 0 ? fill : e;
}
#else
template <int CTRL, int ROWMASK> __device__ __forceinline__ double vmx_dpp_f64(double old, double v) {
    union { double d; int i[2]; } o, s, r; o.d = old; s.d = v;
    r.i[0] = __builtin_amdgcn_update_dpp(o.i[0], s.i[0], CTRL, ROWMASK, 0xf, false);
    r.i[1] = __builtin_amdgcn_update_dpp(o.i[1], s.i[1], CTRL, ROWMASK, 0xf, false);
    return r.d;
}
__device__ __forceinline__ double vmx_wave_incl_max_f64(double v) {
    double t;
    t = vmx_dpp_f64<0x111, 0xf>(VMX_F64_NEG, v); v = t > v ? t : v;
    t = vmx_dpp_f64<0x112, 0xf>(VMX_F64_NEG, v); v = t > v ? t : v;
    t = vmx_dpp_f64<0x114, 0xf>(VMX_F64_NEG, v); v = t > v ? t : v;
    t = vmx_dpp_f64<0x118, 0xf>(VMX_F64_NEG, v); v = t > v ? t : v;
    t = vmx_dpp_f64<0x142, 0xa>(VMX_F64_NEG, v); v = t > v ? t : v;
    t = vmx_dpp_f64<0x143, 0xc>(VMX_F64_NEG, v); v = t > v ? t : v;
// ... 315 lines not shown
```

### vacmap_amd/csrc/vmx_host.h

```cpp
#ifndef VMX_HOST_H
#define VMX_HOST_H
#include "vmx_device.h"
#include "vmx_kernels.h"
#include "../../include/vacmapx.h"
#include <algorithm>
#include <map>
#include <cstring>
#include <string>
#include <vector>
#include <chrono>
#include <atomic>
#include <mutex>
#include <execinfo.h>

namespace vmx {

void set_error(const std::string& s);
int hip_fail(hipError_t e, const char* what, const char* file, int line);

#define VMX_HIP(expr)                                                              \
    do {                                                                           \
        hipError_t _e = (expr);                                                    \
        if (_e != hipSuccess) return vmx::hip_fail(_e, #expr, __FILE__, __LINE__);  \
    } while (0)
// ... 170 lines not shown
    VMX_TRY(b.reserve(bytes));
    vmx::copy_census().add(file, line, bytes);
    const vmx_push_piece pc{b.p, host, bytes};
    return vmx_push_pieces(c, &pc, 1);
}
struct vmx_push_req { vmx::DevBuf* b; const void* host; size_t bytes; };
static inline int vmx_push_many(vm_ctx* c, const vmx_push_req* rq, int np) {
    vmx_push_piece pc[4];
    for (int i = 0; i < np; ++i) { VMX_TRY(rq[i].b->reserve(rq[i].bytes ? rq[i].bytes : 1)); pc[i] = vmx_push_piece{rq[i].b->p, rq[i].host, rq[i].bytes}; }
    return vmx_push_pieces(c, pc, np);
}
template <class T> int vmx_push_to(vm_ctx* c, void* dev, const T* host, size_t n) {
    if (!n) return 0;
    const vmx_push_piece pc{dev, host, sizeof(T) * n};
    return vmx_push_pieces(c, &pc, 1);
}
int vmx_fetch_bytes(vm_ctx* c, void* host, const void* dev, size_t bytes);
template <class T> int vmx_fetch(vm_ctx* c, T* host, const void* dev, size_t n, int line = __builtin_LINE(), const char* file = __builtin_FILE()) {
    if (!n) return 0;
    if (!c->mb.on) return vmx::download(host, dev, n, c->stream, line, file);
    vmx::copy_census().add(file, -line, sizeof(T) * n);
    return vmx_fetch_bytes(c, (void*)host, dev, sizeof(T) * n);
}
struct vmx_fetch_scope {
    vm_ctx* c;
    explicit vmx_fetch_scope(vm_ctx* ctx) : c(ctx) { drop(); }
    ~vmx_fetch_scope() { drop(); }
    void drop() { c->mb.pend.clear(); c->mb.dn_used = 0; c->mb.big_used = 0; }
};

struct vmx_fork {
    vm_ctx* c; int used = 0;
    explicit vmx_fork(vm_ctx* ctx) : c(ctx) { (void)hipEventRecord(c->fork_ev, c->stream); }
    hipStream_t next() {
        hipStream_t s = c->aux[used & 3];
        if (used < 4) (void)hipStreamWaitEvent(s, c->fork_ev, 0);
        ++used;
        return s;
    }
    void join() {
        const int n = used < 4 ? used : 4;
        for (int i = 0; i < n; ++i) { (void)hipEventRecord(c->join_ev[i], c->aux[i]); (void)hipStreamWaitEvent(c->stream, c->join_ev[i], 0); }
        used = 0;
    }
};

__global__ void k_encode(const char* in, uint8_t* out, int64_t n);
__global__ void k_edit_distance(const uint8_t* qcodes, const int64_t* q_off, const uint8_t* tcodes, const int64_t* t_off,
                                int8_t* carry_pool, const int32_t* order, const int32_t* range, int32_t* counters, int which, int64_t* out,
                                int64_t carry_stride, int32_t* oflow);
__global__ void k_size_order(const int64_t* size, const int32_t* n_ptr, int64_t thresh, int32_t* order, int32_t* range, int32_t* counters);
__global__ void k_size_hist(const int64_t* size, const int32_t* n_ptr, int64_t thresh, int32_t* ghist);
__global__ void k_size_scatter(const int64_t* size, const int32_t* n_ptr, const int32_t* ghist, int32_t* gcur, int32_t* order, int32_t* range, int32_t* counters);
static inline void vmx_size_order_wide(vm_ctx* c, const int64_t* size, const int32_t* n_ptr, int64_t n_upper, int64_t thresh, int32_t* order, int32_t* range, int32_t* counters,
                                       int32_t* scratch) {
    static const bool one_wg = getenv("VMX_SIZE_ORDER_ONE") != nullptr;
    if (one_wg) { hipLaunchKernelGGL(k_size_order, dim3(1), dim3(1024), 0, c->stream, size, n_ptr, thresh, order, range, counters); return; }
    (void)hipMemsetAsync(scratch, 0, 4 * 513, c->stream);
    const unsigned G = (unsigned)std::max<int64_t>(1, std::min<int64_t>((n_upper + 1023) / 1024, (int64_t)c->num_cu * 2));
    hipLaunchKernelGGL(k_size_hist, dim3(G), dim3(256), 0, c->stream, size, n_ptr, thresh, scratch);
    hipLaunchKernelGGL(k_size_scatter, dim3(G), dim3(256), 0, c->stream, size, n_ptr, (const int32_t*)scratch, scratch + 257, order, range, counters);
}
__global__ void k_ed_banded(const uint8_t* qcodes, const int64_t* q_off, const uint8_t* tcodes, const int64_t* t_off, const int32_t* order,
                            const int32_t* range, int32_t* counter, int64_t* ub_out);
struct vmx_ext_args;
__global__ void k_ed_banded4(const uint8_t* qcodes, const int64_t* q_off, const uint8_t* tcodes, const int64_t* t_off, const int32_t* order,
                             const int32_t* range, int32_t* counter, int64_t* ub_out);
__global__ void k_ed_flag(const int64_t* ub, const int64_t* q_off, const int64_t* t_off, const int32_t* n_ptr, double maxdiv, int64_t* sizes,
                          int64_t* ed_out, int32_t* n_flagged, int first, const int32_t* prob_read, struct vmx_ext_read* er);
__global__ void k_extend(const uint8_t* tcodes, const int64_t* t_off, const uint8_t* qcodes, const int64_t* q_off, int n_prob,
                         int match, int mismatch, int o, int e, int bw_in, int zdrop, int32_t* out_te, int32_t* out_qe, int32_t* out_sc, const int32_t* n_ptr);
__global__ void k_gapfill_fill(const uint8_t* tcodes, const uint8_t* qcodes, const vmx_dp_prob* probs, int n_prob, int match,
                               int mismatch, int o1, int e1, int o2, int e2, uint8_t* tb_pool, int32_t* bnd_pool, int32_t* out_score,
                               const int32_t* order, int32_t* counter);
__global__ void k_gapfill_fill_ns(const uint8_t* tcodes, const uint8_t* qcodes, vmx_dp_prob* probs, int n_prob, int match,
                                  int mismatch, int o1, int e1, int o2, int e2, uint8_t* tb_pool, int32_t* bnd_pool, int32_t* out_score,
                                  const int32_t* order, const int32_t* range, int32_t* counter, int32_t* redo_list, int32_t* redo_cnt, int ad_pct,
                                  unsigned long long* redo_bytes, const int32_t* n_ptr = nullptr, unsigned long long redo_cap = ~0ULL, int tb_by_ns = 0);
__global__ void k_gapfill_redo(const uint8_t* tcodes, const uint8_t* qcodes, const vmx_dp_prob* probs, int match, int mismatch, int o1, int e1, int o2, int e2,
                               uint8_t* tb_pool, int32_t* bnd_pool, int32_t* out_score, int32_t* redo_list, int32_t* redo_cnt, uint8_t* redo_pool);
static inline int vmx_ad_pct_env(int mode = 0) {
    int pct = mode == 1 ? 40 : 90, pmin = mode == 1 ? 40 : VMX_AD_PCT_MIN_DEFAULT;
    if (const char* e = getenv("VMX_AD_PCT")) { const int v = atoi(e); if (v >= 0 && v <= 60000) pct = v; }
    if (const char* e = getenv("VMX_AD_PCT_MIN")) { const int v = atoi(e); if (v >= 0 && v <= 60000) pmin = v; }
    return pct | (pmin << 16);
}
__global__ void k_gapfill_trace(const uint8_t* tcodes, const uint8_t* qcodes, const vmx_dp_prob* probs, int n_prob, int eqx,
                                const uint8_t* tb_pool, uint32_t* run_pool, char* cig_pool, int32_t* cig_len, const int32_t* band_flag, const uint8_t* redo_pool, int spread, int32_t* cig_q, const int32_t* n_ptr = nullptr);
__global__ void k_flip_sort(const int64_t* rows, const int64_t* aoff, const int64_t* readlens, int n_reads, uint64_t* key_pool,
                            const int64_t* key_off, vmx_anchor* sorted, int32_t* need_reverse);
__global__ void k_chain_global(const vmx_anchor* anchors, const int64_t* aoff, const int32_t* rlist, int nlist, int lds_cap,
                               vmx_tables tab, const double* gapcost_list, double oskipcost, int omaxdiff, int maxgap,
                               double* S_out, int32_t* P_out, int32_t* SA_out, uint8_t* cov_pool, int64_t* gmax_out, int64_t* opcount_out, int rmode,
                               double* FP_pool, double* PP_pool);
static inline int64_t vmx_rows_misfit(const int64_t* rows, int64_t n) {
    for (int64_t i = 0; i < n; ++i) {
        const int64_t q = rows[4 * i], s = rows[4 * i + 2], l = rows[4 * i + 3];
        if (l < 0 || l > 65535 || q < INT32_MIN || q > INT32_MAX || q + l > INT32_MAX || s < INT16_MIN || s > INT16_MAX) return i;
    }
    return -1;
}
__global__ void k_chain_global_rows(const vmx_anchor* anchors, const int64_t* aoff, const int32_t* rlist, int nlist, vmx_tables tab, const double* gapcost_list,
                                    double oskipcost, int omaxdiff, int maxgap, double* S_out, int32_t* P_out, int32_t* SA_out, uint8_t* cov_pool,
                                    int64_t* gmax_out, int64_t* opcount_out, int rmode, double* FP_pool, double* PP_pool, unsigned long long* dbg);
__global__ void k_chain_global_rows_w3(const vmx_anchor* anchors, const int64_t* aoff, const int32_t* rlist, int nlist, vmx_tables tab, const double* gapcost_list,
                                       double oskipcost, int omaxdiff, int maxgap, double* S_out, int32_t* P_out, int32_t* SA_out, uint8_t* cov_pool,
// ... 16 lines not shown
```

### vacmap_amd/csrc/vmx_kernels.h

```cpp
#ifndef VMX_KERNELS_H
#define VMX_KERNELS_H
#include <stdint.h>

struct vmx_dp_prob {
    int64_t t_off, q_off;
    int32_t tl, ql;
    int64_t tb_off;
    int64_t bnd_off;
    int64_t run_off;
    int64_t cig_off;
};

struct vmx_anchor {
    int32_t q;
    int16_t l;
    int16_t s;
    int64_t r;
};

struct vmx_slot { uint64_t key; uint32_t start; uint32_t count; };

struct vmx_tables {
    const float* extra; int32_t extra_n;
    const float* readgap_h; const float* readgap_r; const float* large_readgap;
// ... 126 lines not shown
__host__ __device__ static inline int vmx_ad_ns_nd(int tl, int ql, int match, int o1, int e1, int o2, int e2, int pct, int pct_min, int dpn, int ns_lo, int ns_hi) {
    if (tl <= 0 || ql <= 0) return 0;
    const int mn = tl < ql ? tl : ql;
    int dlo, g = 0;
    for (int ns = ns_lo; ns <= ns_hi; ++ns) {
        g = vmx_ad_geom_nd(tl, ql, dpn * ns, &dlo);
        if (g >= 1 && (g > mn || vmx_ad_margin(g, match, o1, e1, o2, e2) * 100 >= (long long)pct * mn)) return ns;
    }
    return (g >= 1 && vmx_ad_margin(g, match, o1, e1, o2, e2) * 100 >= (long long)pct_min * mn) ? ns_hi : 0;
}
__host__ __device__ static inline int vmx_ad_ns(int tl, int ql, int match, int o1, int e1, int o2, int e2, int pct, int pct_min) {
    return vmx_ad_ns_nd(tl, ql, match, o1, e1, o2, e2, pct, pct_min, 32, 1, VMX_AD_NS_MAX);
}
#define VMX_AD_PCT_DEFAULT 100
#define VMX_AD_PCT_MIN_DEFAULT 65
#ifdef VMX_EMU
#define VMX_ADW_DPN 36
#else
#define VMX_ADW_DPN 128
#endif
#define VMX_ADW_NS_MIN 2
#define VMX_ADW_PCT 100
#define VMX_ADW_PCT_MIN 65
#define VMX_AD_FLAG 16
#define VMX_PK_FLAG 1
#ifdef VMX_EMU
#define VMX_REDO_PK(tl, ql) ((tl) > 0 && (ql) > 0 && VMX_DP16X4_OK(tl, ql) && (tl) + (ql) >= 120)
#else
#ifndef VMX_REDO_PK_MIN
#define VMX_REDO_PK_MIN 384
#endif
#define VMX_REDO_PK(tl, ql) ((tl) > 0 && (ql) > 0 && VMX_DP16X4_OK(tl, ql) && (tl) + (ql) >= VMX_REDO_PK_MIN)
#endif
#define VMX_PK_TB_BYTES(tl, ql) ((int64_t)(((tl) + 127) / 128) * ((ql) + 127) * 128)
#ifndef VMX_AD_AB
#define VMX_AD_AB 4
#endif
static_assert(VMX_AD_AB == 1 || 64 / VMX_AD_AB <= 16, "a 64-byte line of the anti-diagonal traceback holds at most the 16 lanes of a row per anti-diagonal (1-byte slots): AB = 1, 4 or 8");
#define VMX_AD_TB_OFF(s, l) ((((size_t)(s) & ~(size_t)(VMX_AD_AB - 1)) << 6) + ((size_t)(s) & (VMX_AD_AB - 1)) * (64 / VMX_AD_AB) + ((size_t)(l) / (16 / VMX_AD_AB)) * 64 + ((size_t)(l) % (16 / VMX_AD_AB)) * 4)
#define VMX_AD_TB_BYTES(tl, ql) ((int64_t)(((tl) + (ql) + VMX_AD_AB - 1) & ~(VMX_AD_AB - 1)) * 64)
#define VMX_AD_W(ns) ((ns) <= 0 ? 0 : ((ns) == 1 ? 1 : ((ns) == 2 ? 2 : 4)))
#define VMX_AD_TB_OFF_W(s, l, W) (((size_t)(s) / VMX_AD_AB) * (size_t)(VMX_AD_AB * 16 * (W)) + ((size_t)(l) / (64 / (VMX_AD_AB * (W)))) * 64 + ((size_t)(s) % VMX_AD_AB) * (64 / VMX_AD_AB) + ((size_t)(l) % (64 / (VMX_AD_AB * (W)))) * (W))
#define VMX_AD_TB_BYTES_W(tl, ql, W) ((int64_t)(((tl) + (ql) + VMX_AD_AB - 1) & ~(VMX_AD_AB - 1)) * 16 * (W))
#define VMX_X4_TB_BYTES(tl, ql) ((int64_t)(((tl) + 31) / 32) * VMX_X4_W(ql) * 32)
#define VMX_TB_BYTES(tl, ql) (((tl) > 0 && (ql) > 0) ? (VMX_DP16X4_OK(tl, ql) ? VMX_X4_TB_BYTES(tl, ql) : \
                              VMX_DP16_OK(tl, ql) ? VMX_PK_TB_BYTES(tl, ql) : (int64_t)(((tl) + 63) / 64) * ((ql) + 63) * 64) : 0)
#define VMX_TB_BYTES_NS(tl, ql) (((tl) > 0 && (ql) > 0 && VMX_DP16X4_OK(tl, ql)) ? VMX_AD_TB_BYTES(tl, ql) : VMX_TB_BYTES(tl, ql))
#define VMX_REDO_TB_BYTES(tl, ql) (VMX_REDO_PK(tl, ql) ? VMX_PK_TB_BYTES(tl, ql) : VMX_X4_TB_BYTES(tl, ql))
__device__ __forceinline__ uint8_t* vmx_tb_ptr(const uint8_t* tb_pool, const uint8_t* redo_pool, int64_t off) {
    const unsigned long long base = off >= 0 ? (unsigned long long)tb_pool : (unsigned long long)redo_pool;
    return (uint8_t*)(base + (unsigned long long)(off >= 0 ? off : -off - 1));
}
#define VMX_HEAD_THRESH (((int64_t)1 << 18) - 1)
#define VMX_TB_CHUNK ((int64_t)4 << 30)
#ifdef VMX_EMU
#define VMX_MAX_BATCH_BASES 20000
#define VMX_MAX_BATCH_READS 6
#else
#define VMX_MAX_BATCH_BASES ((int64_t)160 << 20)
#define VMX_MAX_BATCH_READS 16384
#endif
#define VMX_LA_SLOT(len) ((len) / 2 + 4096)
#define VMX_SELECT_LDS 3072
#define VMX_LC_LDS_MAX_DEFAULT 13056
#define VMX_GC_LDS_MAX_DEFAULT 13056
#define VMX_CHAIN_LDS_MAX_SHARED 512
#define VMX_LC_BYTES_PER_ANCHOR 12
#define VMX_GC_BYTES_PER_ANCHOR 12

#endif
```

### vacmap_amd/csrc/vmx_round.h

```cpp
#ifndef VMX_ROUND_H
#define VMX_ROUND_H
#include "vmx_kernels.h"
#include "vmx_extend.h"

#define VMX_MAX_CHUNKS 24
#define VMX_ROUND_WGS 128
#define VMX_ROUND_PART_WORDS (256 * 8 + 8)

struct vmx_round_args {
    const vmx_pair_desc* desc; const int32_t* n_prob;
    int64_t* off[6];
    int64_t* tb_size;
    vmx_dp_prob* probs;
    int64_t* part;
    int32_t* stat_out;
    int64_t* plan_out;
    int64_t tb_limit;
    int64_t cap[4];
    int ad_on, ad_match, ad_o1, ad_e1, ad_o2, ad_e2, ad_pct;
    long long epoch;
};
template <bool DP> __global__ void k_round_prep(vmx_round_args A);

__host__ __device__ __forceinline__ int vmx_round_w(const vmx_round_args& A, long long tl, long long ql) {
    return VMX_AD_W(vmx_ad_ns((int)tl, (int)ql, A.ad_match, A.ad_o1, A.ad_e1, A.ad_o2, A.ad_e2, A.ad_pct & 0xffff, (A.ad_pct >> 16) & 0xffff));
}
__host__ __device__ __forceinline__ long long vmx_round_tb_bytes(const vmx_round_args& A, long long tl, long long ql) {
    const bool small = tl > 0 && ql > 0 && VMX_DP16X4_OK(tl, ql);
    return (small && A.ad_on) ? VMX_AD_TB_BYTES_W(tl, ql, vmx_round_w(A, tl, ql)) : VMX_TB_BYTES_NS(tl, ql);
}
__host__ __device__ __forceinline__ long long vmx_round_key(const vmx_round_args& A, long long tl, long long ql) {
    if (tl <= 0 || ql <= 0) return 0;
    if (!VMX_DP16X4_OK(tl, ql)) {
        const long long b = VMX_TB_BYTES(tl, ql);
        if (b > VMX_HEAD_THRESH) return (b < (1LL << 38) ? b : (1LL << 38)) << 24;
        return b << 23;
    }
    const long long b64 = VMX_AD_TB_BYTES(tl, ql);
    if (!A.ad_on) return b64;
    const int w = vmx_round_w(A, tl, ql);
    return w == 4 ? b64 << 16 : (w == 2 ? b64 << 6 : (w == 1 ? b64 >> 4 : (b64 >> 14) + 1));
}
#endif
```

### vacmap_amd/csrc/vmx_stage.h

```cpp
#ifndef VMX_STAGE_H
#define VMX_STAGE_H
#include "vmx_host.h"

struct vm_index_view {
    const uint8_t* codes; const int64_t* coff; int nseq; int64_t total_len;
    const uint64_t* pos; const vmx_slot* table; int table_bits; int k, w, mid_occ;
};
void vmx_index_view(const vm_index* mi, vm_index_view* v);

struct vmx_preset { const vmx_anchor* chain_desc; int64_t len; };

struct vmx_local_bufs {
    vmx::DevBuf sq, dst, rorder, pc2, stg, si, tg, cntp, fp, pp, prep_ws;
    vmx::DevBuf guide_rows, guide_len, ng_used, ng_total, cnt, cur, tpos, hkey, hkey2, dbg, hval, hq, goff, pcnt, gkey, gq, gr, epoch;
    vmx::DevBuf la_rows, la_ekey, la_sorted, la_off, la_cnt, status, gap, rlist, S, P, SA, chain, chain_len, score, variant;
    int64_t la_pool_rows = 0;
    std::vector<int64_t> h_la_off;
    std::vector<int32_t> h_la_cnt;
    void release() {
        vmx::DevBuf* all[] = {&prep_ws, &sq, &dst, &rorder, &pc2, &stg, &si, &tg, &cntp, &fp, &pp, &dbg, &epoch, &hkey2, &guide_rows, &guide_len, &ng_used, &ng_total, &cnt, &cur, &tpos, &hkey, &hval, &hq, &goff, &pcnt, &gkey, &gq, &gr,
                              &la_rows, &la_ekey, &la_sorted, &la_off, &la_cnt, &status, &gap, &rlist, &S, &P, &SA, &chain, &chain_len, &score, &variant};
        for (auto* b : all) b->release();
    }
};
vmx_local_bufs* vmx_ctx_local_bufs(vm_ctx* c);

struct vmx_batch_bufs {
    vmx::DevBuf seed[13];
    vmx::DevBuf nanc64, aoff, rows, lens, keys, koff, sorted, flip, S, P, SA, cov, gmax, opc, rl, gap, scr, soff, res, plen, prow, ocodes;
    vmx::DevBuf er, coff3, soff2, segA, st, en, segA_s, st_s, en_s, segprob, dup, desc[2], rcount, oflow, probread, tl, ql, toff, qoff, tpool, qpool;
    vmx::DevBuf edout, carry, ext3, dpsz[4], dpoff[4], dptab, tb, tbredo, bnd, run, cig, ciglen, dpscore, rec, blob, bloboff, reccoff, recclen, dupd, totals;
    vmx::DevBuf raw, codes, off, order, qrange, scanpart, scanoff, si, tg, cntp, fp, pp, chunkn, sellist, cigq, statblk, szh, side_codes, side_off, roundpart, gfctl, geotot;
    void release() { vmx::DevBuf* p = (vmx::DevBuf*)this; for (size_t i = 0; i < sizeof(*this) / sizeof(vmx::DevBuf); ++i) p[i].release(); }
};
vmx_batch_bufs* vmx_ctx_batch_bufs(vm_ctx* c);

int vmx_global_stage(vm_ctx* c, vmx_batch_bufs& B, const vm_params* prm, int k, int64_t n, const int64_t* d_roff, const std::vector<int64_t>& h_roff,
                     const std::vector<int64_t>& h_aoff, int rmode, int32_t* d_ran);
static inline void vmx_res_ptrs(vmx_batch_bufs& B, int64_t n, double** score, int32_t** mapq, int32_t** np) {
    *score = B.res.as<double>(); *mapq = (int32_t*)(*score + n + 1); *np = *mapq + n + 1;
}

#define VMX_GF_SLOT (32 + 544)
void vmx_gapfill_chunk(vm_ctx* c, vmx_batch_bufs& B, const vm_score& sc, int ad_pct, int eqx, int p0, int64_t pn, const int32_t* n_ptr, int64_t tb_off0,
                       int32_t* ctl, int32_t* redo_list, int64_t redo_cap, hipEvent_t* ke);

extern "C" int vmx_seed_stage(vm_ctx* c, const vm_index* mi, int check_num, int mid_occ, int64_t n, const uint8_t* d_codes, const int64_t* d_roff, int64_t total_bases,
                   vmx::DevBuf* B, std::vector<int64_t>& h_koff, std::vector<int64_t>& h_nhits, vmx::DevBuf* arena = nullptr, int64_t** rows_out = nullptr);
int vmx_local_stage(vm_ctx* c, const vm_index_view& ix, const vm_params* prm, int64_t n, const uint8_t* d_ocodes, const int64_t* d_roff,
                    const std::vector<int64_t>& h_roff, const vmx_anchor* d_path_rows, const int32_t* d_path_len, const int32_t* d_npaths,
                    const int64_t* d_aoff, const std::vector<int64_t>& h_aoff, const double* d_gscore, vmx_local_bufs& L, bool fast = false);
int vmx_launch_chain_select(vm_ctx* c, int64_t n, const int64_t* h_aoff, vmx::DevBuf& d_list, const vmx_anchor* sorted, const int64_t* d_aoff, const int64_t* d_lens,
                            const double* S, const int32_t* P, const int32_t* SA, const int64_t* gmax, const int32_t* flip, int mode, char* scr, const int64_t* soff,
                            int32_t* d_mapq, double* d_score, int32_t* d_np, int32_t* plen, vmx_anchor* prow);
#endif
```

### vacmap_amd/lib.py

```python
import ctypes as C
import os
import numpy as np

_HERE = os.path.dirname(os.path.abspath(__file__))
DEFAULT_SO = os.environ.get('VACMAPX_LIB') or os.path.join(_HERE, 'libvacmapx.so')

VM_ERR_NO_DEVICE = -2
MODES = {'H': 0, 'L': 1, 'S': 2, 'R': 3, 'asm': 4}


class VmxError(RuntimeError):
    def __init__(self, code, msg):
        super().__init__('vacmapx error %d: %s' % (code, msg))
        self.code = code


class Params(C.Structure):
    _fields_ = [('mode', C.c_int32), ('check_num', C.c_int32), ('mid_occ', C.c_int32), ('global_maxdiff', C.c_int32),
                ('local_maxdiff', C.c_int32), ('local_kmersize', C.c_int32), ('eqx', C.c_int32), ('hardclip', C.c_int32),
                ('nodiscard', C.c_int32), ('reserved', C.c_int32), ('global_skipcost', C.c_double),
                ('local_skipcost', C.c_double), ('maxdivergence', C.c_double)]


class Score(C.Structure):
    _fields_ = [('match', C.c_int32), ('mismatch', C.c_int32), ('o1', C.c_int32), ('e1', C.c_int32), ('o2', C.c_int32), ('e2', C.c_int32)]


class CigarOut(C.Structure):
    _fields_ = [('cigar', C.c_void_p), ('q_e', C.c_int32), ('t_e', C.c_int32), ('score', C.c_int32)]


class ChainsOut(C.Structure):
    _fields_ = [('need_reverse', C.POINTER(C.c_int32)), ('mapq', C.POINTER(C.c_int32)), ('score', C.POINTER(C.c_double)),
                ('fast_used', C.POINTER(C.c_int32)), ('read_path_off', C.POINTER(C.c_int64)), ('path_off', C.POINTER(C.c_int64)),
                ('path_anchors', C.POINTER(C.c_int64)), ('S', C.POINTER(C.c_double)), ('P', C.POINTER(C.c_int64)),
                ('S_arg', C.POINTER(C.c_int64)), ('gmax', C.POINTER(C.c_int64)), ('opcount', C.POINTER(C.c_int64))]


class LinkedOut(C.Structure):
    _fields_ = [('gmax', C.c_int64), ('n_hot', C.c_int64), ('n_cold', C.c_int64), ('opcount', C.c_int64), ('cold_max', C.c_double),
                ('S', C.POINTER(C.c_double)), ('P', C.POINTER(C.c_int64)), ('S_arg_hot', C.POINTER(C.c_int64)),
                ('carry_status', C.c_int32), ('saved', C.c_int32), ('n_carry', C.c_int64), ('carry_S', C.POINTER(C.c_double)),
                ('carry_P', C.POINTER(C.c_int64)), ('carry_rows', C.POINTER(C.c_int64)), ('carry_g_max_scores', C.c_double), ('carry_prereadloc', C.c_int64)]


class LocalOut(C.Structure):
    _fields_ = [('status', C.POINTER(C.c_int32)), ('variant', C.POINTER(C.c_int32)), ('score', C.POINTER(C.c_double)),
                ('chain_off', C.POINTER(C.c_int64)), ('chain', C.POINTER(C.c_int64)), ('raw_off', C.POINTER(C.c_int64)),
                ('raw', C.POINTER(C.c_int64))]


class Record(C.Structure):
    _fields_ = [('read_idx', C.c_int32), ('contig', C.c_int32), ('strand', C.c_int32), ('mapq', C.c_int32),
                ('q_st', C.c_int64), ('q_en', C.c_int64), ('r_st', C.c_int64), ('r_en', C.c_int64),
                ('cigar_off', C.c_int64), ('cigar_len', C.c_int64)]


class SamOpts(C.Structure):
    _fields_ = [('md', C.c_int32), ('shortcs', C.c_int32), ('cigar2cg', C.c_int32), ('markunbalancetra', C.c_int32), ('hardclip', C.c_int32),
                ('fakecigar', C.c_int32), ('rg_id', C.c_char_p), ('asm_mode', C.c_int32)]


class BatchStats(C.Structure):
    _fields_ = [(n, C.c_int64) for n in ('n_reads', 'read_bases', 'n_minimizers', 'n_hits', 'n_anchors', 'n_local_hits', 'n_local_anchors',
                                          'n_segments', 'n_ed_problems', 'ed_cells', 'n_ext_problems', 'ext_cells', 'n_dp_problems',
                                          'dp_cells', 'n_records', 'cigar_bytes', 'aligned_bases', 'n_unmapped', 'n_failed',
                                          'dp_string_bytes')] + \
               [('ms_total', C.c_double), ('ms_stage', C.c_double * 16), ('ms_gapfill_fill', C.c_double), ('ms_gapfill_trace', C.c_double),
                ('n_gapfill_launches', C.c_int64), ('n_ed_full', C.c_int64), ('n_ed_tier2', C.c_int64), ('n_ed_tier1', C.c_int64),
                ('n_dp_redo', C.c_int64), ('dp_redo_tb_bytes', C.c_int64), ('ms_local_seed', C.c_double), ('ms_cluster', C.c_double), ('n_host_syncs', C.c_int64), ('n_local_general', C.c_int64), ('n_ext_retries', C.c_int64), ('n_batch_retries', C.c_int64),
                ('n_dp_redo_wide', C.c_int64), ('n_dp_redo_full', C.c_int64)]


def _b(s):
    return s if isinstance(s, (bytes, bytearray)) else s.encode()


def _cat(seqs):
    bs = [_b(s) for s in seqs]
    off = np.zeros(len(bs) + 1, np.int64)
    if bs:
        off[1:] = np.cumsum([len(b) for b in bs])
    return b''.join(bs), off


def _seq_ptrs(seqs):
    keep, ptrs, lens = [], [], []
    for x in seqs:
        if isinstance(x, np.ndarray):
            a = np.ascontiguousarray(x, dtype=np.uint8)
            keep.append(a); ptrs.append(a.ctypes.data); lens.append(a.size)
        else:
            b = C.create_string_buffer(_b(x), len(x)) if len(x) else C.create_string_buffer(1)
            keep.append(b); ptrs.append(C.addressof(b)); lens.append(len(x))
    n = len(ptrs)
    arr = (C.c_void_p * max(n, 1))(*ptrs)
    return keep, C.cast(arr, C.POINTER(C.c_char_p)), (C.c_int64 * max(n, 1))(*lens)


class VmxLib:

    def __init__(self, path=None):
        path = path or DEFAULT_SO
        try:
            if os.environ.get('VACMAPX_SKIP_TORCH') == '1' and 'torch' not in __import__('sys').modules:
                raise ImportError('single-GPU command line: no torch, the library brings the system HIP runtime (saves ~1.5 s of start-up)')
            import torch
        except ImportError:
            pass
        if not os.path.exists(path):
            raise FileNotFoundError('%s not built: run `python -m vacmap_amd.build` (hipcc, gfx950). No fallback exists.' % path)
        L = self.L = C.CDLL(path)
        vp, i32, i64, dbl, cp, P = C.c_void_p, C.c_int32, C.c_int64, C.c_double, C.c_char_p, C.POINTER
        L.vm_last_error.restype = cp
        L.vm_version.restype = cp
        L.vm_free.argtypes = [vp]
        L.vm_params_default.argtypes = [P(Params), C.c_int]
        L.vm_ctx_create.argtypes = [C.c_int, P(vp)]
        L.vm_ctx_destroy.argtypes = [vp]
        L.vm_ctx_set_inflight.argtypes = [vp, C.c_int]
        L.vm_ctx_set_blocking_sync.argtypes = [vp, C.c_int]
        L.vm_debug_chain_counters.argtypes = [C.c_int, C.POINTER(C.c_ulonglong)]
        L.vm_ctx_mem_info.argtypes = [vp, P(i64), P(i64)]
        L.vm_table.argtypes = [vp, C.c_int, P(vp)]; L.vm_table.restype = i64
        L.vm_edit_distance_batch.argtypes = [vp, i64, cp, vp, cp, vp, P(P(i64))]
        L.vm_edit_distance_bound_batch.argtypes = [vp, C.c_int, i64, cp, vp, cp, vp, P(P(i64))]
        L.vm_edit_distance.argtypes = [vp, cp, i64, cp, i64]; L.vm_edit_distance.restype = i64
        L.vm_k_extend_batch.argtypes = [vp] + [C.c_int] * 6 + [i64, cp, vp, cp, vp, P(P(i32)), P(P(i32)), P(P(i32))]
        L.vm_k_cigar_batch.argtypes = [vp, P(Score), C.c_int, i64, cp, vp, cp, vp, P(vp), P(P(i64)), P(P(i32))]
        L.vm_k_cigar.argtypes = [vp, cp, i64, cp, i64, P(Score), C.c_int, C.c_int, C.c_int, P(CigarOut)]
        L.vm_k_cigar_batch_banded.argtypes = [vp, P(Score), C.c_int, i64, cp, vp, cp, vp, P(vp), P(P(i64)), P(P(i32)), vp]
        L.vm_chain_global_batch.argtypes = [vp, P(Params), C.c_int, i64, vp, vp, vp, C.c_int, P(ChainsOut)]
        L.vm_chain_linked.argtypes = [vp, C.c_int, C.c_int, C.c_double, C.c_int, C.c_int, i64, vp, i64, vp, vp, C.c_double, i64, i64, P(LinkedOut)]
        L.vm_linked_out_free.argtypes = [P(LinkedOut)]
        L.vm_align_asm.argtypes = [vp, vp, P(Params), C.c_char_p, i64, i64, i64, i64, P(P(Record)), P(i64), P(vp), P(C.c_int32)]
        L.vm_chains_out_free.argtypes = [P(ChainsOut)]
        L.vm_index_build_fasta.argtypes = [vp, cp, C.c_int, C.c_int, P(vp)]
        L.vm_index_build_mem.argtypes = [vp, C.c_int, P(cp), P(cp), P(i64), C.c_int, C.c_int, P(vp)]
        L.vm_index_save.argtypes = [vp, cp]; L.vm_index_load.argtypes = [vp, cp, P(vp)]
        L.vm_index_save_mmi.argtypes = [vp, cp, C.c_int]; L.vm_index_load_mmi.argtypes = [vp, cp, P(vp)]
        L.vm_index_free.argtypes = [vp]
        for f in ('vm_index_k', 'vm_index_w', 'vm_index_nseq', 'vm_index_mid_occ', 'vm_index_blob_count'):
            getattr(L, f).argtypes = [vp]
        L.vm_index_n_minimizers.argtypes = [vp]; L.vm_index_n_minimizers.restype = i64
        L.vm_index_n_distinct.argtypes = [vp]; L.vm_index_n_distinct.restype = i64
        L.vm_index_seq_info.argtypes = [vp, C.c_int, P(cp), P(i64), P(i64)]
        L.vm_index_seq.argtypes = [vp, C.c_int, i64, i64, vp]; L.vm_index_seq.restype = i64
        L.vm_index_minimizers.argtypes = [vp, P(P(C.c_uint64)), P(P(C.c_uint64)), P(i64)]
        L.vm_index_blob.argtypes = [vp, C.c_int, P(vp), P(i64)]
        L.vm_index_meta_size.argtypes = [vp, P(i64)]; L.vm_index_meta_get.argtypes = [vp, vp, i64]
        L.vm_index_from_meta.argtypes = [vp, vp, i64, P(vp)]
        L.vm_sketch_batch.argtypes = [vp, C.c_int, C.c_int, i64, cp, vp, P(P(C.c_uint64)), P(P(i32)), P(P(C.c_int8)), P(P(i64))]
        L.vm_map_batch.argtypes = [vp, vp, C.c_int, C.c_int, i64, cp, vp, P(P(i64)), P(P(i64))]
        L.vm_map.argtypes = [vp, vp, cp, i64, C.c_int, C.c_int, P(P(i64)), P(i64)]
        L.vm_local_chain_batch.argtypes = [vp, vp, P(Params), i64, cp, vp, vp, vp, vp, P(LocalOut)]
        L.vm_local_out_free.argtypes = [P(LocalOut)]
        L.vm_align_batch.argtypes = [vp, vp, P(Params), i64, cp, vp, P(P(Record)), P(i64), P(vp), vp, P(BatchStats)]
        L.vm_align_trace.argtypes = [vp, vp, P(Params), i64, cp, vp, C.c_int, P(P(i64)), P(P(i64))]
        L.vm_sam_emit.argtypes = [vp, P(SamOpts), i64, vp, vp, vp, vp, vp, vp, vp, vp, vp, i64, vp, vp, C.c_int, P(vp), P(P(i64)), P(i64), P(i64)]
        L.vm_sam_emit_device.argtypes = [vp, vp, P(SamOpts), i64, vp, vp, vp, vp, vp, vp, vp, i64, vp, vp, P(vp), P(P(i64)), P(i64), P(i64)]
        L.vm_sam_emit_device_times.argtypes = [vp, P(dbl)]
        L.vm_blob_gather.argtypes = [vp, vp, vp, i64, vp, vp]; L.vm_blob_gather.restype = i64
        L.vm_blob_write_parts.argtypes = [C.c_int, vp, vp, vp, vp, i64]; L.vm_blob_write_parts.restype = i64
        L.vm_pinned_alloc.argtypes = [i64, C.c_int]; L.vm_pinned_alloc.restype = vp
        L.vm_pinned_free.argtypes = [vp]; L.vm_pinned_free.restype = None
        L.vm_blob_gather_parts.argtypes = [vp, vp, vp, vp, i64, vp]; L.vm_blob_gather_parts.restype = i64
        L.vm_blob_write_parts_mmap.argtypes = [C.c_int, i64, vp, vp, vp, vp, i64, C.c_int]; L.vm_blob_write_parts_mmap.restype = i64
        L.vm_fastx_open.argtypes = [cp, P(vp)]; L.vm_fastx_close.argtypes = [vp]; L.vm_fastx_open_range.argtypes = [cp, i64, i64, P(vp)]
        L.vm_fastx_read.argtypes = [vp, i64, i64] + [P(vp), P(P(i64))] * 4; L.vm_fastx_read.restype = i64
        L.vm_reads_upload.argtypes = [vp, i64, cp, vp, P(vp)]
        L.vm_reads_free.argtypes = [vp]
        L.vm_reads_reupload.argtypes = [vp, vp, i64, vp, vp]
        L.vm_align_resident.argtypes = [vp, vp, P(Params), vp, P(P(Record)), P(i64), P(vp), vp, P(BatchStats)]
        L.vm_bam_writer_create.argtypes = [vp, cp, i64, P(vp)]
        L.vm_bam_writer_free.argtypes = [vp]; L.vm_bam_writer_free.restype = None
        L.vm_bam_header.argtypes = [vp, P(vp), P(i64)]
        L.vm_bam_encode.argtypes = [vp, cp, i64, P(vp), P(i64)]
        L.vm_bam_compress_parts.argtypes = [vp, vp, vp, vp, vp, i64, P(vp), P(i64)]
        L.vm_bam_sorter_create.argtypes = [vp, i64, P(vp)]
        L.vm_bam_sorter_free.argtypes = [vp]; L.vm_bam_sorter_free.restype = None
        L.vm_bam_sorter_add_parts.argtypes = [vp, vp, vp, vp, vp, i64, P(vp), P(i64)]
        L.vm_bam_sorter_plan.argtypes = [vp, vp, i64, i64, P(i64)]
        L.vm_bam_sorter_chunk.argtypes = [vp, i64, P(vp), P(i64)]
        L.vm_bam_sorter_index.argtypes = [vp, P(vp), P(i64)]
# ... 71 lines not shown
        a = np.ctypeslib.as_array(ptr, shape=(max(int(n), 1),))[:int(n)].astype(dtype, copy=True)
        self.lib.L.vm_free(ptr)
        return a

    def table(self, which):
        p = C.c_void_p()
        n = self.lib.check(self.lib.L.vm_table(self.h, which, C.byref(p)))
        ty = C.c_float if which < 4 else C.c_double
        a = np.ctypeslib.as_array(C.cast(p, C.POINTER(ty)), shape=(n,)).copy()
        self.lib.L.vm_free(p)
        return a

    def edit_distance_batch(self, queries, targets):
        q, qo = _cat(queries); t, to = _cat(targets)
        out = C.POINTER(C.c_int64)()
        self.lib.check(self.lib.L.vm_edit_distance_batch(self.h, len(queries), q, qo.ctypes.data, t, to.ctypes.data, C.byref(out)))
        return self._take(out, len(queries), np.int64)

    def edit_distance_bound_batch(self, queries, targets, tier=2):
        q, qo = _cat(queries); t, to = _cat(targets)
        out = C.POINTER(C.c_int64)()
        self.lib.check(self.lib.L.vm_edit_distance_bound_batch(self.h, tier, len(queries), q, qo.ctypes.data, t, to.ctypes.data, C.byref(out)))
        return self._take(out, len(queries), np.int64)

    def edit_distance(self, q, t):
        q, t = _b(q), _b(t)
        return self.lib.check(self.lib.L.vm_edit_distance(self.h, q, len(q), t, len(t)))

    def k_extend_batch(self, targets, queries, match=2, mismatch=-4, o=4, e=4, bw=100, zdrop=50):
        t, to = _cat(targets); q, qo = _cat(queries)
        te = C.POINTER(C.c_int32)(); qe = C.POINTER(C.c_int32)(); sc = C.POINTER(C.c_int32)()
        n = len(targets)
        self.lib.check(self.lib.L.vm_k_extend_batch(self.h, match, mismatch, o, e, bw, zdrop, n, t, to.ctypes.data, q, qo.ctypes.data,
                                                    C.byref(te), C.byref(qe), C.byref(sc)))
        return self._take(sc, n, np.int32), self._take(te, n, np.int32), self._take(qe, n, np.int32)

    def k_cigar_batch(self, targets, queries, match=2, mismatch=-4, o1=4, e1=2, o2=24, e2=1, eqx=False):
        t, to = _cat(targets); q, qo = _cat(queries)
        n = len(targets)
        sc = Score(match, mismatch, o1, e1, o2, e2)
        cg = C.c_void_p(); co = C.POINTER(C.c_int64)(); ss = C.POINTER(C.c_int32)()
        self.lib.check(self.lib.L.vm_k_cigar_batch(self.h, C.byref(sc), int(eqx), n, t, to.ctypes.data, q, qo.ctypes.data,
                                                   C.byref(cg), C.byref(co), C.byref(ss)))
        off = self._take(co, n + 1, np.int64)
        blob = C.string_at(cg.value, int(off[-1])) if off[-1] else b''
        self.lib.L.vm_free(cg)
        cigars = [blob[off[i]:off[i + 1] - 1].decode() for i in range(n)]
        return cigars, self._take(ss, n, np.int32)

    def k_cigar_batch_banded(self, targets, queries, match=2, mismatch=-4, o1=4, e1=2, o2=24, e2=1, eqx=False):
        t, to = _cat(targets); q, qo = _cat(queries)
        n = len(targets)
        sc = Score(match, mismatch, o1, e1, o2, e2)
        cg = C.c_void_p(); co = C.POINTER(C.c_int64)(); fl = C.POINTER(C.c_int32)(); st = (C.c_int64 * 6)()
        self.lib.check(self.lib.L.vm_k_cigar_batch_banded(self.h, C.byref(sc), int(eqx), n, t, to.ctypes.data, q, qo.ctypes.data,
                                                          C.byref(cg), C.byref(co), C.byref(fl), st))
        off = self._take(co, n + 1, np.int64)
        blob = C.string_at(cg.value, int(off[-1])) if off[-1] else b''
        self.lib.L.vm_free(cg)
        cigars = [blob[off[i]:off[i + 1] - 1].decode() for i in range(n)]
        return cigars, self._take(fl, n, np.int32), {'eligible': st[0], 'proven': st[1], 'redo': st[2], 'not_eligible': st[3],
                                                          'redo_wide': st[4], 'redo_full': st[5]}

    def k_cigar(self, target, query, match=2, mismatch=-4, gap_open_1=4, gap_extend_1=2, gap_open_2=24, gap_extend_2=1,
                bw=-1, zdropvalue=-1, eqx=False):
        t, q = _b(target), _b(query)
        sc = Score(match, mismatch, gap_open_1, gap_extend_1, gap_open_2, gap_extend_2)
        out = CigarOut()
        self.lib.check(self.lib.L.vm_k_cigar(self.h, t, len(t), q, len(q), C.byref(sc), bw, zdropvalue, int(eqx), C.byref(out)))
        cg = C.string_at(out.cigar).decode() if out.cigar else ''
        self.lib.L.vm_free(out.cigar)
        return cg, 0, out.q_e, out.t_e, 0, 0

    def chain_global_batch(self, prm, kmersize, anchors_list, readlens, want_raw=False):
        n = len(anchors_list)
        aoff = np.zeros(n + 1, np.int64)
        for i, a in enumerate(anchors_list):
            aoff[i + 1] = aoff[i] + len(a)
        rows = np.ascontiguousarray(np.concatenate([np.asarray(a, dtype=np.int64).reshape(-1, 4) for a in anchors_list]) if n else np.zeros((0, 4), np.int64))
        rl = np.ascontiguousarray(readlens, dtype=np.int64)
        out = ChainsOut()
        self.lib.check(self.lib.L.vm_chain_global_batch(self.h, C.byref(prm), kmersize, n, rows.ctypes.data, aoff.ctypes.data, rl.ctypes.data,
                                                        int(want_raw), C.byref(out)))
        res = []
        rpo = np.ctypeslib.as_array(out.read_path_off, shape=(n + 1,)).copy()
        npaths = int(rpo[-1])
        po = np.ctypeslib.as_array(out.path_off, shape=(npaths + 1,)).copy()
        nrows = int(po[-1])
        pa = np.ctypeslib.as_array(out.path_anchors, shape=(max(nrows, 1), 4))[:nrows].copy()
        tot = int(aoff[-1])
        for r in range(n):
            d = {'need_reverse': bool(out.need_reverse[r]), 'mapq': int(out.mapq[r]), 'score': float(out.score[r]),
                 'fast_used': bool(out.fast_used[r]), 'gmax': int(out.gmax[r]), 'opcount': int(out.opcount[r]),
                 'paths': [pa[po[p]:po[p + 1]] for p in range(rpo[r], rpo[r + 1])]}
            if want_raw:
                a, b = int(aoff[r]), int(aoff[r + 1])
                d['S'] = np.ctypeslib.as_array(out.S, shape=(max(tot, 1),))[a:b].copy()
                d['P'] = np.ctypeslib.as_array(out.P, shape=(max(tot, 1),))[a:b].copy()
                d['S_arg'] = np.ctypeslib.as_array(out.S_arg, shape=(max(tot, 1),))[a:b].copy()
            res.append(d)
        self.lib.L.vm_chains_out_free(C.byref(out))
        return res

    def sketch_batch(self, k, w, seqs):
        s, off = _cat(seqs)
        n = len(seqs)
        h = C.POINTER(C.c_uint64)(); p = C.POINTER(C.c_int32)(); z = C.POINTER(C.c_int8)(); oo = C.POINTER(C.c_int64)()
        self.lib.check(self.lib.L.vm_sketch_batch(self.h, k, w, n, s, off.ctypes.data, C.byref(h), C.byref(p), C.byref(z), C.byref(oo)))
        o = self._take(oo, n + 1, np.int64)
        m = int(o[-1])
        H = self._take(h, m, np.uint64); Pp = self._take(p, m, np.int32); Z = self._take(z, m, np.int8)
        return [(H[o[i]:o[i + 1]], Pp[o[i]:o[i + 1]], Z[o[i]:o[i + 1]]) for i in range(n)]

    def map(self, index, seq, check_num=100, mid_occ=-1):
        sq = _b(seq)
# ... 617 lines not shown
```

Before: 3.526.

## Order gap-fill queue by band width and exact span for tighter pairing

Replaces the size-class histogram ordering of gap-fill DP problems with a new queue key. Banded problems are keyed by their strip count and exact tl+ql, and each gets its own bin, so problems paired into one wavefront have matching band and length and fewer lanes sit idle. New hist/scatter kernels use a persistent global histogram with last-block prefix sum and self-clearing, moved out of the per-chunk control slot. The fill loop also gains counters for per-task versus owned band steps, which add wave reductions and atomics.

```diff
diff --git a/include/vacmapx.h b/include/vacmapx.h
--- a/include/vacmapx.h
+++ b/include/vacmapx.h
@@ -121,6 +121,8 @@
                      const int64_t* q_off, char** cigars, int64_t** cigar_off, int32_t** scores);
 int vm_k_cigar_batch_banded(vm_ctx*, const vm_score*, int eqx, int64_t n, const char* t, const int64_t* t_off, const char* q,
                             const int64_t* q_off, char** cigars, int64_t** cigar_off, int32_t** band_flag, int64_t* stats);
+int vm_k_gapfill_order(vm_ctx*, int64_t n, const int64_t* keys, int64_t thresh, int32_t* order, int32_t* range, int32_t* counters, int clear_area, int64_t* area_nonzero);
+int64_t vm_gapfill_queue_key(const vm_score*, int ad_pct, int64_t tl, int64_t ql);
 int vm_k_extend_batch(vm_ctx*, int match, int mismatch, int o, int e, int bw, int zdrop, int64_t n, const char* t,
                       const int64_t* t_off, const char* q, const int64_t* q_off, int32_t** t_e, int32_t** q_e, int32_t** score);
 typedef struct vm_cigar_out { char* cigar; int32_t q_e, t_e, score; } vm_cigar_out;
@@ -165,6 +167,8 @@
     int64_t n_batch_retries;
     int64_t n_dp_redo_wide;
     int64_t n_dp_redo_full;
+    int64_t dp_band_task_steps;
+    int64_t dp_band_own_steps;
 } vm_batch_stats;
 
 int vm_align_batch(vm_ctx*, const vm_index*, const vm_params*, int64_t n_reads, const char* seqs, const int64_t* offsets,
diff --git a/vacmap_amd/csrc/k_dp.hip b/vacmap_amd/csrc/k_dp.hip
--- a/vacmap_amd/csrc/k_dp.hip
+++ b/vacmap_amd/csrc/k_dp.hip
@@ -472,6 +472,7 @@
     const bool ad_ok = vmx_ad_scores_ok(match, mismatch, o1, e1, o2, e2);
     const int n_head = range[0] < n_prob ? range[0] : n_prob;
     bool head = n_head > 0;
+    unsigned long long task_steps = 0, own_steps = 0;
     while (true) {
         int pX = -1, pY = -1;
         if (head) {
@@ -499,6 +500,12 @@
             const int gX = (nsX > 0 && fitX) ? vmx_ad_geom(prX.tl, prX.ql, ns, &dloX) : 0, gY = (nsY > 0 && fitY) ? vmx_ad_geom(prY.tl, prY.ql, ns, &dloY) : 0;
             const int tlX = gX > 0 ? prX.tl : 0, qlX = gX > 0 ? prX.ql : 0, tlY = gY > 0 ? prY.tl : 0, qlY = gY > 0 ? prY.ql : 0;
             int scX = 0, scY = 0;
+            {
+                const int afX = tlX > 0 ? tlX + qlX : 0, afY = tlY > 0 ? tlY + qlY : 0;
+                const int own = (lane & 15) == 0 ? ((afX + 1) >> 1) * nsX + ((afY + 1) >> 1) * nsY : 0;
+                task_steps += (unsigned long long)(unsigned)(((vmx_uniform_i32(vmx_wave_max_i32(afX > afY ? afX : afY)) + 1) >> 1) * ns);
+                own_steps += (unsigned long long)(unsigned)vmx_uniform_i32(vmx_wave_sum_i32(own));
+            }
 #define VMX_AD_RUN(NSV) vmx_gapfill_fill_ad<NSV>(tcodes + prX.t_off, qcodes + prX.q_off, tlX, qlX, dloX, tb_pool + prX.tb_off, tcodes + prY.t_off, qcodes + prY.q_off, tlY, qlY, dloY, \
                                                  tb_pool + prY.tb_off, match, mismatch, o1, e1, o2, e2, lane, scX, scY)
             if (ns == 1) VMX_AD_RUN(1); else if (ns == 2) VMX_AD_RUN(2); else if (ns == 3) VMX_AD_RUN(3); else VMX_AD_RUN(4);
@@ -533,6 +540,7 @@
             vmx_gapfill_fill_one<false>(tcodes, qcodes, probs, p, match, mismatch, o1, e1, o2, e2, tb_pool, bnd_pool, out_score, lane);
         }
     }
+    if (lane == 0 && task_steps) { atomicAdd((unsigned long long*)(redo_cnt + 8), task_steps); atomicAdd((unsigned long long*)(redo_cnt + 10), own_steps); }
 }
 
 __global__ void __launch_bounds__(64) k_gapfill_fill(const uint8_t* __restrict__ tcodes, const uint8_t* __restrict__ qcodes,
diff --git a/vacmap_amd/csrc/k_ed.hip b/vacmap_amd/csrc/k_ed.hip
--- a/vacmap_amd/csrc/k_ed.hip
+++ b/vacmap_amd/csrc/k_ed.hip
@@ -1,13 +1,6 @@
 #include "vmx_device.h"
 #include "vmx_kernels.h"
 
-__device__ __forceinline__ int vmx_size_class(long long s) {
-    if (s < 0) return -1;
-    if (s == 0) return 0;
-    const int e = 63 - __clzll(s);
-    const int m = (int)((e >= 2 ? s >> (e - 2) : s << (2 - e)) & 3);
-    return (e << 2) | m;
-}
 __global__ void __launch_bounds__(1024) k_size_order(const int64_t* __restrict__ size, const int32_t* __restrict__ n_ptr, int64_t thresh,
                                                      int32_t* __restrict__ order, int32_t* __restrict__ range, int32_t* __restrict__ counters) {
     VMX_SETPRIO(3);
diff --git a/vacmap_amd/csrc/k_gf_order.hip b/vacmap_amd/csrc/k_gf_order.hip
--- /dev/null
+++ b/vacmap_amd/csrc/k_gf_order.hip
@@ -0,0 +1,93 @@
+#include "vmx_device.h"
+#include "vmx_kernels.h"
+
+#ifdef VMX_EMU
+#define VMX_GFQ_LD(p) __atomic_load_n((p), __ATOMIC_RELAXED)
+#define VMX_GFQ_DONE(p) __atomic_fetch_add((p), 1, __ATOMIC_ACQ_REL)
+#else
+#define VMX_GFQ_LD(p) __hip_atomic_load((p), __ATOMIC_RELAXED, __HIP_MEMORY_SCOPE_AGENT)
+#define VMX_GFQ_DONE(p) __hip_atomic_fetch_add((p), 1, __ATOMIC_ACQ_REL, __HIP_MEMORY_SCOPE_AGENT)
+#endif
+
+__device__ __forceinline__ int vmx_gfq_slot(long long key) {
+    if (key < 0) return -1;
+    if ((key >> 24) == 1) {
+        const int ns = (int)(key >> 16) & 0xff, s = (int)key & 0xffff;
+        if (ns >= 1 && ns <= VMX_AD_NS_MAX && s >= 1 && s <= VMX_DP16X4_MAX) return VMX_GFQ_TAIL + (ns - 1) * VMX_DP16X4_MAX + (s - 1);
+    }
+    const int c = vmx_size_class(key);
+    return c < VMX_GFQ_TAIL ? c : c + VMX_GFQ_BINS;
+}
+
+__global__ void __launch_bounds__(256) k_gfq_hist(const int64_t* __restrict__ key, const int32_t* __restrict__ n_ptr, int64_t thresh, int32_t* __restrict__ G,
+                                                  int32_t* __restrict__ range, int32_t* __restrict__ counters) {
+    __shared__ int s_h[VMX_GFQ_SLOTS + 1];
+    __shared__ int s_w[4];
+    __shared__ int s_last;
+    const int n = *n_ptr, tid = (int)threadIdx.x, lane = vmx_lane(), wv = tid >> 6;
+    for (int t = tid; t <= VMX_GFQ_SLOTS; t += 256) s_h[t] = 0;
+    __syncthreads();
+    int nl = 0;
+    for (int i = (int)(blockIdx.x * 256) + tid; i < n; i += (int)(gridDim.x * 256)) {
+        const long long k = key[i];
+        const int sl = vmx_gfq_slot(k);
+        if (k > thresh) ++nl;
+        if (sl >= 0) atomicAdd(&s_h[sl], 1);
+    }
+    if (nl) atomicAdd(&s_h[VMX_GFQ_SLOTS], nl);
+    __syncthreads();
+    for (int t = tid; t <= VMX_GFQ_SLOTS; t += 256) if (s_h[t]) atomicAdd(&G[t], s_h[t]);
+    __syncthreads();
+    if (tid == 0) {
+        __threadfence();
+        s_last = VMX_GFQ_DONE(&G[VMX_GFQ_SLOTS + 1]) + 1 == (int)gridDim.x;
+    }
+    __syncthreads();
+    if (!s_last) return;
+    constexpr int PER = (VMX_GFQ_SLOTS + 255) / 256;
+    int cnt[PER], sum = 0;
+#pragma unroll
+    for (int u = 0; u < PER; ++u) { const int sl = VMX_GFQ_SLOTS - 1 - (tid * PER + u); cnt[u] = sl >= 0 ? VMX_GFQ_LD(&G[sl]) : 0; sum += cnt[u]; }
+    const int inc = vmx_wave_incl_scan_i32(sum);
+    if (lane == 63) s_w[wv] = inc;
+    __syncthreads();
+    int base = inc - sum;
+    for (int w = 0; w < wv; ++w) base += s_w[w];
+#pragma unroll
+    for (int u = 0; u < PER; ++u) { const int sl = VMX_GFQ_SLOTS - 1 - (tid * PER + u); if (sl >= 0) G[sl] = base; base += cnt[u]; }
+    if (tid == 0) {
+        range[0] = VMX_GFQ_LD(&G[VMX_GFQ_SLOTS]); range[1] = s_w[0] + s_w[1] + s_w[2] + s_w[3];
+        counters[0] = 0; counters[1] = 0; counters[2] = 0; counters[3] = 0;
+        G[VMX_GFQ_SLOTS] = 0; G[VMX_GFQ_SLOTS + 1] = 0;
+    }
+}
+
+__global__ void __launch_bounds__(256) k_gfq_scatter(const int64_t* __restrict__ key, const int32_t* __restrict__ n_ptr, int32_t* __restrict__ G, int32_t* __restrict__ order) {
+    VMX_SETPRIO(3);
+    __shared__ int s_c[VMX_GFQ_SLOTS];
+    __shared__ int s_last;
+    const int n = *n_ptr, tid = (int)threadIdx.x;
+    for (int t = tid; t < VMX_GFQ_SLOTS; t += 256) s_c[t] = 0;
+    __syncthreads();
+    for (int i = (int)(blockIdx.x * 256) + tid; i < n; i += (int)(gridDim.x * 256)) {
+        const int sl = vmx_gfq_slot(key[i]);
+        if (sl >= 0) atomicAdd(&s_c[sl], 1);
+    }
+    __syncthreads();
+    for (int t = tid; t < VMX_GFQ_SLOTS; t += 256) if (s_c[t]) s_c[t] = atomicAdd(&G[t], s_c[t]);
+    __syncthreads();
+    for (int i = (int)(blockIdx.x * 256) + tid; i < n; i += (int)(gridDim.x * 256)) {
+        const int sl = vmx_gfq_slot(key[i]);
+        if (sl < 0) continue;
+        const int at = atomicAdd(&s_c[sl], 1);
+        if ((unsigned)at < (unsigned)n) order[at] = i;
+    }
+    __syncthreads();
+    if (tid == 0) {
+        __threadfence();
+        s_last = VMX_GFQ_DONE(&G[VMX_GFQ_SLOTS + 2]) + 1 == (int)gridDim.x;
+    }
+    __syncthreads();
+    if (!s_last) return;
+    for (int t = tid; t < VMX_GFQ_WORDS; t += 256) G[t] = 0;
+}
diff --git a/vacmap_amd/csrc/vmx_align.hip b/vacmap_amd/csrc/vmx_align.hip
--- a/vacmap_amd/csrc/vmx_align.hip
+++ b/vacmap_amd/csrc/vmx_align.hip
@@ -166,17 +166,17 @@
 }
 
 void vmx_gapfill_chunk(vm_ctx* c, vmx_batch_bufs& B, const vm_score& sc, int ad_pct, int eqx, int p0, int64_t pn, const int32_t* n_ptr, int64_t tb_off0,
-                       int32_t* ctl, int32_t* redo_list, int64_t redo_cap, hipEvent_t* ke) {
+                       int32_t* ctl, int32_t* qhist, int32_t* redo_list, int64_t redo_cap, hipEvent_t* ke) {
     int fill_waves = 16;
     if (const char* e = getenv("VMX_FILL_WAVES")) { const int v = atoi(e); if (v >= 1 && v <= 32) fill_waves = v; }
     static const int tr_spread = [] { const char* e = getenv("VMX_TRACE_SPREAD"); const int v = e ? atoi(e) : 1; return v >= 1 && v <= 64 ? v : 1; }();
     int32_t* d_range = ctl; int32_t* d_cnt = ctl + 4; int32_t* d_redo_cnt = ctl + 12;
-    unsigned long long* d_redo_bytes = (unsigned long long*)(ctl + 16); int32_t* scratch = ctl + 32;
+    unsigned long long* d_redo_bytes = (unsigned long long*)(ctl + 16);
     uint8_t* tb_base = B.tb.as<uint8_t>() - tb_off0;
     vmx_dp_prob* probs = B.dptab.as<vmx_dp_prob>() + p0; int32_t* score = B.dpscore.as<int32_t>() + p0;
     const unsigned Gs = (unsigned)std::max<int64_t>(1, std::min<int64_t>((pn + 1023) / 1024, (int64_t)c->num_cu * 2));
-    hipLaunchKernelGGL(k_size_hist, dim3(Gs), dim3(256), 0, c->stream, B.dpsz[0].as<int64_t>() + p0, n_ptr, (int64_t)((1LL << 42) - 1), scratch);
-    hipLaunchKernelGGL(k_size_scatter, dim3(Gs), dim3(256), 0, c->stream, B.dpsz[0].as<int64_t>() + p0, n_ptr, (const int32_t*)scratch, scratch + 257, B.order.as<int32_t>(), d_range, d_cnt);
+    hipLaunchKernelGGL(k_gfq_hist, dim3(Gs), dim3(256), 0, c->stream, B.dpsz[0].as<int64_t>() + p0, n_ptr, (int64_t)((1LL << 42) - 1), qhist, d_range, d_cnt);
+    hipLaunchKernelGGL(k_gfq_scatter, dim3(Gs), dim3(256), 0, c->stream, B.dpsz[0].as<int64_t>() + p0, n_ptr, qhist, B.order.as<int32_t>());
     if (ke) (void)hipEventRecord(ke[0], c->stream);
     {
         vmx_lowprio lp(c);
@@ -469,7 +469,7 @@
     VMX_TRY(B.recclen.reserve(4 * (size_t)(cS + 1))); VMX_TRY(B.dupd.reserve((size_t)cB + 64));
     VMX_HIP(hipMemsetAsync(B.oflow.p, 0, 4, c->stream));
     VMX_TRY(B.statblk.reserve(2048)); VMX_HIP(hipMemsetAsync(B.statblk.p, 0, 2048, c->stream));
-    const size_t gfctl_bytes = (size_t)2 * (VMX_MAX_CHUNKS + 1) * VMX_GF_SLOT * 4;
+    const size_t gfctl_slots = (size_t)2 * (VMX_MAX_CHUNKS + 1) * VMX_GF_SLOT, gfctl_bytes = (gfctl_slots + VMX_GFQ_WORDS) * 4;
     VMX_TRY(B.gfctl.reserve(gfctl_bytes)); VMX_HIP(hipMemsetAsync(B.gfctl.p, 0, gfctl_bytes, c->stream));
     vmx_ext_args A; memset(&A, 0, sizeof A);
     A.n_reads = (int)n; A.nseq = ix.nseq; A.local_maxdiff = preset ? 50 : prm->local_maxdiff ; A.asm_long = preset ? 1 : 0; A.nodiscard = prm->nodiscard; A.hardclip = prm->hardclip; A.redo_only = 0; A.mode = prm->mode; A.maxdivergence = prm->maxdivergence;
@@ -530,7 +530,7 @@
     auto gf_chunk = [&](int pass, int q, int p0, int64_t pn, const int32_t* n_ptr, int64_t tb_off0) {
         int32_t* ctl = B.gfctl.as<int32_t>() + (size_t)(pass * (VMX_MAX_CHUNKS + 1) + q) * VMX_GF_SLOT;
         hipEvent_t* ke = q < 8 ? c->gev + (pass ? 24 : 0) + 3 * q : nullptr;
-        vmx_gapfill_chunk(c, B, gf_score, ad_pct, prm->eqx, p0, pn, n_ptr, tb_off0, ctl, B.order.as<int32_t>() + round_cap + 32, gf_redo_cap, ke);
+        vmx_gapfill_chunk(c, B, gf_score, ad_pct, prm->eqx, p0, pn, n_ptr, tb_off0, ctl, B.gfctl.as<int32_t>() + gfctl_slots, B.order.as<int32_t>() + round_cap + 32, gf_redo_cap, ke);
         if (ke) c->n_gev[pass] = q + 1;
         gf_chunks[pass] = q + 1;
     };
@@ -651,7 +651,7 @@
     VMX_TRY(vmx_fetch(c, fin, B.statblk.as<int64_t>() + 32, 14));
     int64_t geo[8] = {0, 0, 0, 0, 0, 0, 0, 0};
     if (fast_local) VMX_TRY(vmx_fetch(c, geo, B.geotot.p, 6));
-    std::vector<int32_t> h_ctl(gfctl_bytes / 4);
+    std::vector<int32_t> h_ctl(gfctl_slots);
     VMX_TRY(vmx_fetch(c, h_ctl.data(), B.gfctl.p, h_ctl.size()));
     VMX_TRY(vmx_fetch(c, er.data(), B.er.p, (size_t)n)); VMX_TRY(vmx_fetch(c, h_gmax.data(), B.gmax.p, (size_t)n));
     VMX_TRY(vmx_fetch(c, *recs, B.totals.p, (size_t)g_nr)); VMX_TRY(vmx_fetch(c, *cigar_blob, B.dupd.p, (size_t)g_nb));
@@ -665,14 +665,15 @@
         if (geo[5] && getenv("VMX_DBG_POOLS")) fprintf(stderr, "[pools] extend stage: %lld read(s) did not fit the history-sized pools (run again alone)\n", (long long)geo[5]);
     }
     {
-        bool again = false; int64_t need_max = 0, ad_failed = 0;
+        bool again = false; int64_t need_max = 0, ad_failed = 0, band_own = 0;
         for (int pass = 0; pass < 2; ++pass)
             for (int q = 0; q < gf_chunks[pass]; ++q) {
                 const int32_t* ctl = h_ctl.data() + (size_t)(pass * (VMX_MAX_CHUNKS + 1) + q) * VMX_GF_SLOT;
                 unsigned long long rb = 0; memcpy(&rb, ctl + 16, 8);
-                st.n_dp_redo += ctl[12]; st.n_dp_redo_wide += ctl[18]; st.n_dp_redo_full += ctl[19]; st.dp_redo_tb_bytes += (int64_t)rb; st.dp_cells += (int64_t)rb; ad_failed += ctl[15];
+                st.n_dp_redo += ctl[12]; st.n_dp_redo_wide += ctl[18]; st.n_dp_redo_full += ctl[19]; { unsigned long long ts = 0, os = 0; memcpy(&ts, ctl + 20, 8); memcpy(&os, ctl + 22, 8); st.dp_band_task_steps += (int64_t)ts; band_own += (int64_t)os; } st.dp_redo_tb_bytes += (int64_t)rb; st.dp_cells += (int64_t)rb; ad_failed += ctl[15];
                 need_max = std::max<int64_t>(need_max, (int64_t)rb);
             }
+        st.dp_band_own_steps += band_own / 8;
         c->redo_need_max = std::max<long long>(c->redo_need_max, need_max);
         if (need_max > gf_redo_cap) { again = true; if (getenv("VMX_DBG_POOLS")) fprintf(stderr, "[pools] gap fill: a chunk's second launch needs %.3f GB of traceback space, the pool held %.3f: running the batch again\n", need_max / 1e9, gf_redo_cap / 1e9); }
         if (again) return VMX_RETRY_BATCH;
@@ -782,7 +783,7 @@
             tot.ms_total += st.ms_total; for (int i = 0; i < 16; ++i) tot.ms_stage[i] += st.ms_stage[i];
             tot.ms_gapfill_fill += st.ms_gapfill_fill; tot.ms_gapfill_trace += st.ms_gapfill_trace; tot.n_gapfill_launches += st.n_gapfill_launches;
             tot.n_ed_full += st.n_ed_full; tot.n_ed_tier2 += st.n_ed_tier2; tot.n_ed_tier1 += st.n_ed_tier1;
-            tot.n_dp_redo += st.n_dp_redo; tot.n_dp_redo_wide += st.n_dp_redo_wide; tot.n_dp_redo_full += st.n_dp_redo_full; tot.dp_redo_tb_bytes += st.dp_redo_tb_bytes; tot.ms_local_seed += st.ms_local_seed; tot.ms_cluster += st.ms_cluster; tot.n_host_syncs += st.n_host_syncs; tot.n_local_general += st.n_local_general; tot.n_ext_retries += st.n_ext_retries; tot.n_batch_retries += st.n_batch_retries;
+            tot.n_dp_redo += st.n_dp_redo; tot.n_dp_redo_wide += st.n_dp_redo_wide; tot.n_dp_redo_full += st.n_dp_redo_full; tot.dp_band_task_steps += st.dp_band_task_steps; tot.dp_band_own_steps += st.dp_band_own_steps; tot.dp_redo_tb_bytes += st.dp_redo_tb_bytes; tot.ms_local_seed += st.ms_local_seed; tot.ms_cluster += st.ms_cluster; tot.n_host_syncs += st.n_host_syncs; tot.n_local_general += st.n_local_general; tot.n_ext_retries += st.n_ext_retries; tot.n_batch_retries += st.n_batch_retries;
         }
     }
     *recs = (vm_record*)malloc(sizeof(vm_record) * std::max<size_t>(all.size(), 1)); *cigar_blob = (char*)malloc(std::max<size_t>(blob.size(), 1));
diff --git a/vacmap_amd/csrc/vmx_capi.hip b/vacmap_amd/csrc/vmx_capi.hip
--- a/vacmap_amd/csrc/vmx_capi.hip
+++ b/vacmap_amd/csrc/vmx_capi.hip
@@ -539,8 +539,8 @@
     VMX_TRY(B.run.reserve(sizeof(uint32_t) * (size_t)(run + 4))); VMX_TRY(B.cig.reserve((size_t)cig + 16));
     VMX_TRY(B.ciglen.reserve(4 * (size_t)(n + 1))); VMX_TRY(B.cigq.reserve(4 * (size_t)(n + 1))); VMX_TRY(B.dpscore.reserve(4 * (size_t)(n + 1)));
     VMX_TRY(B.order.reserve(4 * (size_t)(2 * n + 64)));
-    VMX_TRY(B.gfctl.reserve(4 * VMX_GF_SLOT)); VMX_HIP(hipMemsetAsync(B.gfctl.p, 0, 4 * VMX_GF_SLOT, c->stream));
-    if (n) vmx_gapfill_chunk(c, B, *sc, ad_pct, eqx, 0, n, B.chunkn.as<int32_t>(), 0, B.gfctl.as<int32_t>(), B.order.as<int32_t>() + n + 32, redo, nullptr);
+    VMX_TRY(B.gfctl.reserve(4 * (VMX_GF_SLOT + VMX_GFQ_WORDS))); VMX_HIP(hipMemsetAsync(B.gfctl.p, 0, 4 * (VMX_GF_SLOT + VMX_GFQ_WORDS), c->stream));
+    if (n) vmx_gapfill_chunk(c, B, *sc, ad_pct, eqx, 0, n, B.chunkn.as<int32_t>(), 0, B.gfctl.as<int32_t>(), B.gfctl.as<int32_t>() + VMX_GF_SLOT, B.order.as<int32_t>() + n + 32, redo, nullptr);
     std::vector<char> hc((size_t)cig + 16); std::vector<int32_t> hl((size_t)n), flag((size_t)n), ctl(32);
     VMX_TRY(download(hc.data(), B.cig.p, (size_t)cig, c->stream));
     VMX_TRY(download(hl.data(), B.ciglen.p, (size_t)n, c->stream));
@@ -555,10 +555,44 @@
         small += sm; nb += sm && flag[i] > VMX_AD_FLAG;
         eligible += sm && vmx_ad_ns(probs[i].tl, probs[i].ql, sc->match, sc->o1, sc->e1, sc->o2, sc->e2, ad_pct & 0xffff, (ad_pct >> 16) & 0xffff) > 0;
     }
-    if (stats) { stats[0] = eligible; stats[1] = nb; stats[2] = ctl[12]; stats[3] = n - small; stats[4] = ctl[18]; stats[5] = ctl[19]; }
+    unsigned long long task_steps = 0, own_steps = 0; memcpy(&task_steps, &ctl[20], 8); memcpy(&own_steps, &ctl[22], 8);
+    if (stats) { stats[0] = eligible; stats[1] = nb; stats[2] = ctl[12]; stats[3] = n - small; stats[4] = ctl[18]; stats[5] = ctl[19]; stats[6] = (int64_t)task_steps; stats[7] = (int64_t)(own_steps / 8); }
     if (band_flag) { *band_flag = host_alloc<int32_t>((size_t)n); memcpy(*band_flag, flag.data(), sizeof(int32_t) * (size_t)n); }
     cigar_strings(n, probs.data(), hc.data(), hl.data(), cigars, cigar_off);
     return VM_OK;
+}
+
+int vm_k_gapfill_order(vm_ctx* c, int64_t n, const int64_t* keys, int64_t thresh, int32_t* order, int32_t* range, int32_t* counters, int clear_area, int64_t* area_nonzero) {
+    if (!c) { set_error("no context"); return VM_ERR_NO_CTX; }
+    if (n < 0 || n > 0x7fffffff) { set_error("vm_k_gapfill_order: bad problem count"); return VM_ERR_ARG; }
+    VMX_HIP(hipSetDevice(c->device));
+    vmx_batch_bufs& B = *vmx_ctx_batch_bufs(c);
+    const int32_t nn = (int32_t)n;
+    VMX_TRY(upload(B.dpsz[0], keys, (size_t)n, c->stream)); VMX_TRY(upload(B.chunkn, &nn, 1, c->stream));
+    VMX_TRY(B.order.reserve(4 * (size_t)(n + 64))); VMX_HIP(hipMemsetAsync(B.order.p, 0xff, 4 * (size_t)(n + 64), c->stream));
+    const size_t words = VMX_GF_SLOT + VMX_GFQ_WORDS;
+    VMX_TRY(B.gfctl.reserve(4 * words)); VMX_HIP(hipMemsetAsync(B.gfctl.p, 0, 4 * (clear_area ? words : (size_t)VMX_GF_SLOT), c->stream));
+    int32_t* ctl = B.gfctl.as<int32_t>(); int32_t* G = ctl + VMX_GF_SLOT;
+    VMX_HIP(hipMemsetAsync(ctl + 4, 0xff, 16, c->stream));
+    const unsigned Gs = (unsigned)std::max<int64_t>(1, std::min<int64_t>((n + 1023) / 1024, (int64_t)c->num_cu * 2));
+    hipLaunchKernelGGL(k_gfq_hist, dim3(Gs), dim3(256), 0, c->stream, B.dpsz[0].as<int64_t>(), B.chunkn.as<int32_t>(), thresh, G, ctl, ctl + 4);
+    hipLaunchKernelGGL(k_gfq_scatter, dim3(Gs), dim3(256), 0, c->stream, B.dpsz[0].as<int64_t>(), B.chunkn.as<int32_t>(), G, B.order.as<int32_t>());
+    std::vector<int32_t> h(words);
+    VMX_TRY(download(order, B.order.p, (size_t)n, c->stream));
+    VMX_TRY(download(h.data(), B.gfctl.p, words, c->stream));
+    VMX_HIP(vmx_stream_sync(c));
+    VMX_HIP(hipGetLastError());
+    range[0] = h[0]; range[1] = h[1];
+    for (int i = 0; i < 4; ++i) counters[i] = h[4 + i];
+    int64_t nz = 0;
+    for (size_t i = VMX_GF_SLOT; i < words; ++i) nz += h[i] != 0;
+    if (area_nonzero) *area_nonzero = nz;
+    return VM_OK;
+}
+int64_t vm_gapfill_queue_key(const vm_score* sc, int ad_pct, int64_t tl, int64_t ql) {
+    vmx_round_args R; memset(&R, 0, sizeof R);
+    R.ad_on = 1; R.ad_match = sc->match; R.ad_o1 = sc->o1; R.ad_e1 = sc->e1; R.ad_o2 = sc->o2; R.ad_e2 = sc->e2; R.ad_pct = ad_pct;
+    return vmx_round_key(R, tl, ql);
 }
 
 int vm_k_cigar(vm_ctx* c, const char* t, int64_t tl, const char* q, int64_t ql, const vm_score* sc, int bw, int zdrop, int eqx, vm_cigar_out* out) {
diff --git a/vacmap_amd/csrc/vmx_device.h b/vacmap_amd/csrc/vmx_device.h
--- a/vacmap_amd/csrc/vmx_device.h
+++ b/vacmap_amd/csrc/vmx_device.h
@@ -129,6 +129,14 @@
     union { double d; int i[2]; } u; u.d = v;
     u.i[0] = vmx_readlane(u.i[0], l); u.i[1] = vmx_readlane(u.i[1], l);
     return u.d;
+}
+
+__device__ __forceinline__ int vmx_size_class(long long s) {
+    if (s < 0) return -1;
+    if (s == 0) return 0;
+    const int e = 63 - __clzll(s);
+    const int m = (int)((e >= 2 ? s >> (e - 2) : s << (2 - e)) & 3);
+    return (e << 2) | m;
 }
 
 __device__ __forceinline__ int vmx_wave_max_i32(int v) {
diff --git a/vacmap_amd/csrc/vmx_host.h b/vacmap_amd/csrc/vmx_host.h
--- a/vacmap_amd/csrc/vmx_host.h
+++ b/vacmap_amd/csrc/vmx_host.h
@@ -246,6 +246,8 @@
 __global__ void k_size_order(const int64_t* size, const int32_t* n_ptr, int64_t thresh, int32_t* order, int32_t* range, int32_t* counters);
 __global__ void k_size_hist(const int64_t* size, const int32_t* n_ptr, int64_t thresh, int32_t* ghist);
 __global__ void k_size_scatter(const int64_t* size, const int32_t* n_ptr, const int32_t* ghist, int32_t* gcur, int32_t* order, int32_t* range, int32_t* counters);
+__global__ void k_gfq_hist(const int64_t* key, const int32_t* n_ptr, int64_t thresh, int32_t* G, int32_t* range, int32_t* counters);
+__global__ void k_gfq_scatter(const int64_t* key, const int32_t* n_ptr, int32_t* G, int32_t* order);
 static inline void vmx_size_order_wide(vm_ctx* c, const int64_t* size, const int32_t* n_ptr, int64_t n_upper, int64_t thresh, int32_t* order, int32_t* range, int32_t* counters,
                                        int32_t* scratch) {
     static const bool one_wg = getenv("VMX_SIZE_ORDER_ONE") != nullptr;
diff --git a/vacmap_amd/csrc/vmx_kernels.h b/vacmap_amd/csrc/vmx_kernels.h
--- a/vacmap_amd/csrc/vmx_kernels.h
+++ b/vacmap_amd/csrc/vmx_kernels.h
@@ -202,6 +202,12 @@
     return (uint8_t*)(base + (unsigned long long)(off >= 0 ? off : -off - 1));
 }
 #define VMX_HEAD_THRESH (((int64_t)1 << 18) - 1)
+#define VMX_GFQ_BAND_KEY(ns, s) (((int64_t)1 << 24) | ((int64_t)(ns) << 16) | (int64_t)(s))
+#define VMX_GFQ_BINS (VMX_AD_NS_MAX * VMX_DP16X4_MAX)
+#define VMX_GFQ_TAIL 16
+#define VMX_GFQ_SLOTS (256 + VMX_GFQ_BINS)
+#define VMX_GFQ_WORDS (VMX_GFQ_SLOTS + 3)
+static_assert(VMX_DP16X4_MAX < (1 << 16) && VMX_AD_NS_MAX < (1 << 8), "fields of the band problems' queue key");
 #define VMX_TB_CHUNK ((int64_t)4 << 30)
 #ifdef VMX_EMU
 #define VMX_MAX_BATCH_BASES 20000
diff --git a/vacmap_amd/csrc/vmx_round.h b/vacmap_amd/csrc/vmx_round.h
--- a/vacmap_amd/csrc/vmx_round.h
+++ b/vacmap_amd/csrc/vmx_round.h
@@ -22,9 +22,10 @@
 };
 template <bool DP> __global__ void k_round_prep(vmx_round_args A);
 
-__host__ __device__ __forceinline__ int vmx_round_w(const vmx_round_args& A, long long tl, long long ql) {
-    return VMX_AD_W(vmx_ad_ns((int)tl, (int)ql, A.ad_match, A.ad_o1, A.ad_e1, A.ad_o2, A.ad_e2, A.ad_pct & 0xffff, (A.ad_pct >> 16) & 0xffff));
+__host__ __device__ __forceinline__ int vmx_round_ns(const vmx_round_args& A, long long tl, long long ql) {
+    return vmx_ad_ns((int)tl, (int)ql, A.ad_match, A.ad_o1, A.ad_e1, A.ad_o2, A.ad_e2, A.ad_pct & 0xffff, (A.ad_pct >> 16) & 0xffff);
 }
+__host__ __device__ __forceinline__ int vmx_round_w(const vmx_round_args& A, long long tl, long long ql) { return VMX_AD_W(vmx_round_ns(A, tl, ql)); }
 __host__ __device__ __forceinline__ long long vmx_round_tb_bytes(const vmx_round_args& A, long long tl, long long ql) {
     const bool small = tl > 0 && ql > 0 && VMX_DP16X4_OK(tl, ql);
     return (small && A.ad_on) ? VMX_AD_TB_BYTES_W(tl, ql, vmx_round_w(A, tl, ql)) : VMX_TB_BYTES_NS(tl, ql);
@@ -38,7 +39,7 @@
     }
     const long long b64 = VMX_AD_TB_BYTES(tl, ql);
     if (!A.ad_on) return b64;
-    const int w = vmx_round_w(A, tl, ql);
-    return w == 4 ? b64 << 16 : (w == 2 ? b64 << 6 : (w == 1 ? b64 >> 4 : (b64 >> 14) + 1));
+    const int ns = vmx_round_ns(A, tl, ql);
+    return ns > 0 ? VMX_GFQ_BAND_KEY(ns, tl + ql) : (b64 >> 14) + 1;
 }
 #endif
diff --git a/vacmap_amd/csrc/vmx_stage.h b/vacmap_amd/csrc/vmx_stage.h
--- a/vacmap_amd/csrc/vmx_stage.h
+++ b/vacmap_amd/csrc/vmx_stage.h
@@ -41,9 +41,9 @@
     *score = B.res.as<double>(); *mapq = (int32_t*)(*score + n + 1); *np = *mapq + n + 1;
 }
 
-#define VMX_GF_SLOT (32 + 544)
+#define VMX_GF_SLOT 32
 void vmx_gapfill_chunk(vm_ctx* c, vmx_batch_bufs& B, const vm_score& sc, int ad_pct, int eqx, int p0, int64_t pn, const int32_t* n_ptr, int64_t tb_off0,
-                       int32_t* ctl, int32_t* redo_list, int64_t redo_cap, hipEvent_t* ke);
+                       int32_t* ctl, int32_t* qhist, int32_t* redo_list, int64_t redo_cap, hipEvent_t* ke);
 
 extern "C" int vmx_seed_stage(vm_ctx* c, const vm_index* mi, int check_num, int mid_occ, int64_t n, const uint8_t* d_codes, const int64_t* d_roff, int64_t total_bases,
                    vmx::DevBuf* B, std::vector<int64_t>& h_koff, std::vector<int64_t>& h_nhits, vmx::DevBuf* arena = nullptr, int64_t** rows_out = nullptr);
diff --git a/vacmap_amd/lib.py b/vacmap_amd/lib.py
--- a/vacmap_amd/lib.py
+++ b/vacmap_amd/lib.py
@@ -69,7 +69,7 @@
                [('ms_total', C.c_double), ('ms_stage', C.c_double * 16), ('ms_gapfill_fill', C.c_double), ('ms_gapfill_trace', C.c_double),
                 ('n_gapfill_launches', C.c_int64), ('n_ed_full', C.c_int64), ('n_ed_tier2', C.c_int64), ('n_ed_tier1', C.c_int64),
                 ('n_dp_redo', C.c_int64), ('dp_redo_tb_bytes', C.c_int64), ('ms_local_seed', C.c_double), ('ms_cluster', C.c_double), ('n_host_syncs', C.c_int64), ('n_local_general', C.c_int64), ('n_ext_retries', C.c_int64), ('n_batch_retries', C.c_int64),
-                ('n_dp_redo_wide', C.c_int64), ('n_dp_redo_full', C.c_int64)]
+                ('n_dp_redo_wide', C.c_int64), ('n_dp_redo_full', C.c_int64), ('dp_band_task_steps', C.c_int64), ('dp_band_own_steps', C.c_int64)]
 
 
 def _b(s):
@@ -130,6 +130,8 @@
         L.vm_k_cigar_batch.argtypes = [vp, P(Score), C.c_int, i64, cp, vp, cp, vp, P(vp), P(P(i64)), P(P(i32))]
         L.vm_k_cigar.argtypes = [vp, cp, i64, cp, i64, P(Score), C.c_int, C.c_int, C.c_int, P(CigarOut)]
         L.vm_k_cigar_batch_banded.argtypes = [vp, P(Score), C.c_int, i64, cp, vp, cp, vp, P(vp), P(P(i64)), P(P(i32)), vp]
+        L.vm_k_gapfill_order.argtypes = [vp, i64, vp, i64, vp, vp, vp, C.c_int, P(i64)]
+        L.vm_gapfill_queue_key.argtypes = [P(Score), C.c_int, i64, i64]; L.vm_gapfill_queue_key.restype = i64
         L.vm_chain_global_batch.argtypes = [vp, P(Params), C.c_int, i64, vp, vp, vp, C.c_int, P(ChainsOut)]
         L.vm_chain_linked.argtypes = [vp, C.c_int, C.c_int, C.c_double, C.c_int, C.c_int, i64, vp, i64, vp, vp, C.c_double, i64, i64, P(LinkedOut)]
         L.vm_linked_out_free.argtypes = [P(LinkedOut)]
@@ -307,7 +309,7 @@
         t, to = _cat(targets); q, qo = _cat(queries)
         n = len(targets)
         sc = Score(match, mismatch, o1, e1, o2, e2)
-        cg = C.c_void_p(); co = C.POINTER(C.c_int64)(); fl = C.POINTER(C.c_int32)(); st = (C.c_int64 * 6)()
+        cg = C.c_void_p(); co = C.POINTER(C.c_int64)(); fl = C.POINTER(C.c_int32)(); st = (C.c_int64 * 8)()
         self.lib.check(self.lib.L.vm_k_cigar_batch_banded(self.h, C.byref(sc), int(eqx), n, t, to.ctypes.data, q, qo.ctypes.data,
                                                           C.byref(cg), C.byref(co), C.byref(fl), st))
         off = self._take(co, n + 1, np.int64)
@@ -315,7 +317,17 @@
         self.lib.L.vm_free(cg)
         cigars = [blob[off[i]:off[i + 1] - 1].decode() for i in range(n)]
         return cigars, self._take(fl, n, np.int32), {'eligible': st[0], 'proven': st[1], 'redo': st[2], 'not_eligible': st[3],
-                                                          'redo_wide': st[4], 'redo_full': st[5]}
+                                                          'redo_wide': st[4], 'redo_full': st[5], 'band_task_steps': st[6], 'band_own_steps': st[7]}
+
+    def k_gapfill_order(self, keys, thresh=(1 << 42) - 1, clear_area=True):
+        keys = np.ascontiguousarray(keys, dtype=np.int64)
+        n = len(keys)
+        order = np.empty(max(n, 1), np.int32); rng = np.zeros(2, np.int32); ctr = np.zeros(4, np.int32); nz = C.c_int64(-1)
+        self.lib.check(self.lib.L.vm_k_gapfill_order(self.h, n, keys.ctypes.data, int(thresh), order.ctypes.data, rng.ctypes.data, ctr.ctypes.data, int(clear_area), C.byref(nz)))
+        return order[:int(rng[1])].copy(), rng, ctr, int(nz.value)
+
+    def gapfill_queue_key(self, tl, ql, ad_pct, match=2, mismatch=-4, o1=4, e1=2, o2=24, e2=1):
+        return int(self.lib.L.vm_gapfill_queue_key(C.byref(Score(match, mismatch, o1, e1, o2, e2)), int(ad_pct), int(tl), int(ql)))
 
     def k_cigar(self, target, query, match=2, mismatch=-4, gap_open_1=4, gap_extend_1=2, gap_open_2=24, gap_extend_2=1,
                 bw=-1, zdropvalue=-1, eqx=False):
```

Measured after the change: 3.463. 0.982x the previous value.
